# johnnyjana730/MVIN

Hardware: AMD Instinct MI355X
Metric: (user,item) pairs scored/sec @ dim=64 hop=2 fan-out=32; % HBM roofline (higher is better)
Workload: dtype f32

## Files before the change

mvin_amd/csrc/mvin_abi.hip:

```cpp
#include <cstdlib>
#include <cstdarg>
#include <cstdio>
#include <string>

#include "mvin_kernels.h"
#include "mvin_fused_agg.h"

namespace {

thread_local std::string g_last_error;

int fail(int code, const char* fmt, ...) {
    char buf[512];
    va_list ap;
    va_start(ap, fmt);
    vsnprintf(buf, sizeof(buf), fmt, ap);
    va_end(ap);
    g_last_error = buf;
    return code;
}

int hip_result(hipError_t e, const char* what) {
    if (e == hipSuccess) return 0;
    fail((int)e, "%s: %s", what, hipGetErrorString(e));
    return (int)e;
}

bool bad_dim(int D) { return D < 4 || D > MVIN_MAX_DIM || (D & 3) != 0; }

size_t geom_sum(int B, int K, int from, int to) {
    size_t s = 0, p = 1;
    for (int e = 0; e <= to; ++e) {
        if (e >= from) s += p;
        p *= (size_t)K;
    }
    return s * (size_t)B;
}

struct EntityTableList {
    const float* E;
    int n_entity;
    hipStream_t st;
    hipError_t err = hipSuccess;
    int n = 0;
    mvin::EntityTableJob jobs[mvin::kEtMaxJobs];
    void add(const float* W, int w_nk, float* out) {
        if (n == mvin::kEtMaxJobs) flush();
        jobs[n++] = mvin::EntityTableJob{W, out, w_nk};
    }
    void flush() {
        if (n > 0 && err == hipSuccess) err = mvin::launch_entity_tables(E, n_entity, jobs, n, st);
        n = 0;
    }
};

int build_entity_tables(const char* who, const float* E, int n_entity, const float* relation_kge, int nR, float* er, const float* user_mlp_W,
                        int n_o, float* tw, const float* fold_blk, float* fold_tabs, void* stream) {
    const size_t tab = (size_t)n_entity * 64, DD = (size_t)64 * 64;
    EntityTableList l{E, n_entity, (hipStream_t)stream};
    if (er)
        for (int r = 0; r < nR; ++r) l.add(relation_kge + r * DD, 1, er + r * tab);
    if (tw)
        for (int j = 0; j < n_o; ++j) l.add(user_mlp_W + j * DD, 0, tw + j * tab);
    if (fold_tabs)
        for (int i = 0; i < 4; ++i) l.add(fold_blk + i * DD, 0, fold_tabs + i * tab);
    l.flush();
    return hip_result(l.err, who);
}

}

extern "C" {

int mvin_abi_version(void) { return MVIN_ABI_VERSION; }

int mvin_debug_read_trace(long long* host_dst, size_t n) {
    if (!host_dst) return -1;
    static const bool ka = getenv("MVIN_KA_TRACE") != nullptr;
    static const bool pk = getenv("MVIN_PACK_TRACE") != nullptr;
    if (getenv("MVIN_SMALL_TRACE")) return (int)mvin::small_read_trace(host_dst, n);
    if (getenv("MVIN_KAF_TRACE")) return (int)mvin::kaf_read_trace(host_dst, n);
    if (pk) return (int)mvin::pack_read_prof(host_dst, n);
    if (ka && getenv("MVIN_KA_TRACE")[0] == '2') return (int)mvin::kas_read_trace(host_dst, n);
    return (int)(ka ? mvin::ka_read_trace(host_dst, n) : mvin::split_read_trace(host_dst, n));
}

const char* mvin_last_error(void) { return g_last_error.c_str(); }

size_t mvin_ent_elems(int B, int K, int levels) { return geom_sum(B, K, 0, levels); }

size_t mvin_rel_elems(int B, int K, int levels) { return levels > 0 ? geom_sum(B, K, 1, levels) : 0; }

int mvin_expand_ids(const int32_t* adj_entity, const int32_t* adj_relation, const int64_t* items_i64,
                    const int32_t* items_i32, int B, int K, int levels, int n_entity,
                    int32_t* ent_out, int32_t* rel_out, void* stream) {
    if (!ent_out || (!items_i64 && !items_i32) || (items_i64 && items_i32))
        return fail(-1, "mvin_expand_ids: need ent_out and exactly one of items_i64/items_i32");
    if (levels > 0 && (!adj_entity || !adj_relation || !rel_out))
        return fail(-1, "mvin_expand_ids: null adjacency/rel_out with levels=%d", levels);
    if (B <= 0 || K <= 0 || levels < 0 || n_entity <= 0)
        return fail(-2, "mvin_expand_ids: bad sizes B=%d K=%d levels=%d n_entity=%d", B, K, levels, n_entity);
    return hip_result(mvin::launch_expand(adj_entity, adj_relation, items_i64, items_i32, B, K, levels,
                                          n_entity, ent_out, rel_out, (hipStream_t)stream),
                      "mvin_expand_ids");
}

int mvin_rel_score(const float* relation_emb, const float* urh_weights, int nR, int D, float* t_out,
                   void* stream) {
    if (!relation_emb || !urh_weights || !t_out) return fail(-1, "mvin_rel_score: null pointer");
    if (nR <= 0 || D <= 0) return fail(-2, "mvin_rel_score: bad sizes nR=%d D=%d", nR, D);
    return hip_result(mvin::launch_rel_score(relation_emb, urh_weights, nR, D, t_out, (hipStream_t)stream),
                      "mvin_rel_score");
}

int mvin_linear_fwd(const mvin_linear_args* a, void* stream) {
    if (!a) return fail(-1, "mvin_linear_fwd: null args");
    if (a->nsrc < 1 || a->nsrc > MVIN_MAX_SRC) return fail(-2, "mvin_linear_fwd: nsrc=%d", a->nsrc);
    if (a->Dsrc < 4 || (a->Dsrc & 3) || a->Dout < 1 || a->Dout > MVIN_MAX_DIM)
        return fail(-2, "mvin_linear_fwd: Dsrc=%d (need %%4==0) Dout=%d (need 1..%d)", a->Dsrc, a->Dout,
                    MVIN_MAX_DIM);
    if ((size_t)a->nsrc * a->Dsrc > 4096) return fail(-2, "mvin_linear_fwd: nsrc*Dsrc > 4096");
    if (a->rows < 0) return fail(-2, "mvin_linear_fwd: rows < 0");
    if (!a->out) return fail(-1, "mvin_linear_fwd: null out");
    for (int s = 0; s < a->nsrc; ++s)
        if (!a->src[s]) return fail(-1, "mvin_linear_fwd: null src[%d]", s);
    if (!a->W && ((a->nsrc != 1 && !a->sum_sources) || a->Dsrc != a->Dout))
        return fail(-2, "mvin_linear_fwd: identity (W=NULL) needs nsrc==1 and Dsrc==Dout");
    if (a->ldo < a->Dout) return fail(-2, "mvin_linear_fwd: ldo < Dout");
    if (a->rowbias && a->rows_per_group < 1) return fail(-2, "mvin_linear_fwd: rows_per_group < 1");
    if (a->score_u && a->Dout > (a->sum_sources ? 1 : a->nsrc) * a->Dsrc + 4)
        return fail(-2, "mvin_linear_fwd: fused score needs Dout <= Din + 4");
    if (a->rows == 0) return 0;
    return hip_result(mvin::launch_linear(*a, (hipStream_t)stream), "mvin_linear_fwd");
}

static int agg_common(mvin::GatherAttnArgs& g, int B, int N, int K, int D, const char* who) {
    if (B <= 0 || N <= 0 || K <= 0) return fail(-2, "%s: bad sizes B=%d N=%d K=%d", who, B, N, K);
    if (bad_dim(D)) return fail(-2, "%s: D=%d (need %%4==0, 4..%d)", who, D, MVIN_MAX_DIM);
    if (K > 4096) return fail(-2, "%s: K=%d > 4096", who, K);
    if (!g.self_vec || !g.Wagg || !g.out) return fail(-1, "%s: null self_vec/Wagg/out", who);
    g.T = (int64_t)B * N;
    g.N = N;
    g.K = K;
    g.D = D;
    g.lpr_log2 = mvin::lpr_log2_for(D);
    return 0;
}

int mvin_gather_attn_fwd(const float* table, const int32_t* adj_entity, const int32_t* adj_relation,
                         const int32_t* node_ids, const float* rel_score, const float* self_vec,
                         const float* Wc, const float* c_child, const float* Wagg, const float* bagg, int B,
                         int N, int K, int D, int n_entity, float* out, float* probs, void* stream) {
    return mvin_gather_attn_fwd_ex(table, adj_entity, adj_relation, node_ids, rel_score, self_vec, Wc, c_child,
                                   Wagg, bagg, B, N, K, D, n_entity, out, probs, nullptr, nullptr, 0, stream);
}

int mvin_gather_attn_fwd_ex(const void* table, const int32_t* adj_entity, const int32_t* adj_relation,
                            const int32_t* node_ids, const float* rel_score, const float* self_vec,
                            const float* Wc, const float* c_child, const float* Wagg, const float* bagg, int B,
                            int N, int K, int D, int n_entity, float* out, float* probs, float* s_out,
                            float* z_out, int table_bf16, void* stream) {
    mvin::GatherAttnArgs g{};
    g.table_bf16 = table_bf16 ? 1 : 0;
    g.s_out = s_out;
    g.z_out = z_out;
    g.gather = 1;
    g.table = table;
    g.adj_e = adj_entity;
    g.adj_r = adj_relation;
    g.node_ids = node_ids;
    g.rel_score = rel_score;
    g.self_vec = self_vec;
    g.Wc = Wc;
    g.c_child = c_child;
    g.Wagg = Wagg;
    g.bagg = bagg;
    g.out = out;
    g.probs = probs;
    if (!table || !adj_entity || !node_ids || (rel_score && !adj_relation))
        return fail(-1, "mvin_gather_attn_fwd: null table/adjacency/node_ids");
    if (n_entity <= 0) return fail(-2, "mvin_gather_attn_fwd: n_entity=%d", n_entity);
    if (probs && !rel_score) return fail(-2, "mvin_gather_attn_fwd: probs requested without rel_score");
    if (int rc = agg_common(g, B, N, K, D, "mvin_gather_attn_fwd")) return rc;
    return hip_result(mvin::launch_gather_attn(g, (hipStream_t)stream), "mvin_gather_attn_fwd_ex");
}

int mvin_gather_attn_l2_supported(int D, int K) { return mvin::fused_l2_supported(D, K) ? 1 : 0; }

int mvin_probe_gather_l2(const void* table, const int32_t* child_ids, const int32_t* grandchild_ids, int64_t n_parents, int K,
                         int D, int n_entity, int table_bf16, float* sums, void* stream) {
    const char* who = "mvin_probe_gather_l2";
    if (!table || !child_ids || !grandchild_ids || !sums) return fail(-1, "%s: null pointer", who);
    if (n_parents <= 0 || K <= 0 || n_entity <= 0) return fail(-2, "%s: bad sizes", who);
    const int rb = D * (table_bf16 ? 2 : 4);
    if (!(rb == 64 || rb == 128 || rb == 256 || (rb == 512 && !table_bf16)))
        return fail(-3, "%s: row bytes %d (64, 128, 256 or 512)", who, rb);
    return hip_result(mvin::launch_gather_probe_l2(table, child_ids, grandchild_ids, n_parents, K, D, table_bf16, sums,
                                                   (hipStream_t)stream), who);
}

int mvin_gather_attn_l2_variant(int D, int K, int64_t n_parents, int n_entity, int want_probs) {
    return mvin_gather_attn_l2_variant_ex(D, K, n_parents, n_entity, want_probs, 0);
}

int mvin_gather_attn_l2_variant_ex(int D, int K, int64_t n_parents, int n_entity, int want_probs, int table_bf16) {
    if (!mvin::fused_l2_supported(D, K)) return 0;
    mvin::FusedL2Args f{};
    f.K = K;
    f.P = n_parents;
    f.adj_bytes = (uint64_t)n_entity * (uint64_t)K * 4;
    float probe = 0.f;
    if (want_probs) f.probs_parent = f.probs_child = &probe;
    f.table_bytes = (uint64_t)n_entity * (uint64_t)D * (table_bf16 ? 2 : 4);
    if (mvin::fused_d32_applies(f, D)) return 4;
    if (mvin::fused_l2_split_in_use() && mvin::fused_split_applies(f, D)) return 2;
    return mvin::fused_d16_applies(f, D) ? 3 : 1;
}

static int gather_attn_l2_impl(const void* table, const int32_t* adj_entity, const int32_t* adj_relation,
                               const int32_t* parent_ids, int pid_stride, const float* t0, const float* t1,
                               const float* W1, const float* W2, const float* b1, const float* b2, const float* q,
                               const float* A0, const float* a0, int B, int parents_per_pair, int K, int D,
                               int n_entity, int nR, float* nagg0, float* nagg1, float* probs_parent,
                               float* probs_child, int table_bf16, void* stream, bool encoded = false, bool prj = false,
                               const int32_t* order = nullptr, const float* agg = nullptr) {
    const char* who = prj ? "mvin_gather_attn_l2_prj_fwd" : encoded ? "mvin_gather_attn_l2_enc_fwd" : "mvin_gather_attn_l2_fwd";
    if (prj && (table_bf16 || !W1 || !W2 || !q))
        return fail(-1, "%s: projected tables are fp32 and go with the queries", who);
    if (encoded && !mvin::fused_packed_supported(D, K))
        return fail(-3, "%s: unsupported shape D=%d K=%d (D in {32,64,128}, K in {16,32,64,128})", who, D, K);
    if (!mvin::fused_l2_supported(D, K))
        return fail(-3, "%s: unsupported shape D=%d K=%d (D in {16,32,64,128}, K power of two in [4,256])",
                    who, D, K);
    if (!table || !adj_entity || !parent_ids || !A0 || !nagg0 || !nagg1) return fail(-1, "%s: null pointer", who);
    if ((t0 || t1) && !adj_relation) return fail(-1, "%s: attention needs adj_relation", who);
    if ((W1 == nullptr) != (W2 == nullptr)) return fail(-1, "%s: W1 and W2 must be given together", who);
    if (W1 && !q) return fail(-1, "%s: projection needs the query vectors q", who);
    if ((probs_parent || probs_child) && !t0) return fail(-2, "%s: probs requested without t0", who);
    if (B <= 0 || parents_per_pair <= 0 || n_entity <= 0 || nR <= 0 || nR > 4096)
        return fail(-2, "%s: bad sizes B=%d parents_per_pair=%d n_entity=%d nR=%d", who, B, parents_per_pair,
                    n_entity, nR);
    mvin::FusedL2Args f{};
    f.table = table;
    f.adj_e = adj_entity;
    f.adj_r = adj_relation;
    f.parent_ids = parent_ids;
    f.t0 = t0;
    f.t1 = t1;
    f.W1 = W1;
    f.W2 = W2;
    f.b1 = b1;
    f.b2 = b2;
    f.q = q;
    f.A0 = A0;
    f.a0 = a0;
    f.nagg0 = nagg0;
    f.nagg1 = nagg1;
    f.probs_parent = probs_parent;
    f.probs_child = probs_child;
    f.P = (int64_t)B * parents_per_pair;
    f.table_bytes = (uint64_t)n_entity * (uint64_t)D * (table_bf16 ? 2 : 4);
    f.adj_bytes = (uint64_t)n_entity * (uint64_t)K * 4;
    f.parents_per_pair = parents_per_pair;
    f.K = K;
    f.nR = nR;
    f.pid_stride = pid_stride;
    f.max_id = (unsigned)(n_entity - 1);
    f.prj = prj ? 1 : 0;
    int l = 0;
    if (agg) {
        f.agg = const_cast<float*>(agg);
        f.order = order;
        if (!(prj && encoded && mvin::fused_agg_applies(f, D) && (!order || parents_per_pair == 1)))
            return fail(-3, "mvin_gather_attn_l2_agg_fwd: D = 64, K in {16, 32, 64}, n_entity <= 2^24, tables < 1 GiB, adjacency and outputs < 2 GiB "
                            "(a parent order: one parent per pair)");
        return hip_result(mvin::launch_gather_attn_l2_agg(f, (hipStream_t)stream), "mvin_gather_attn_l2_agg_fwd");
    }
    if (order) {
        f.order = order;
        if (!(prj && encoded && parents_per_pair == 1 && mvin::fused_wpp_applies(f, D)))
            return fail(-3, "%s: a parent order is taken by the wave-per-parent kernel only (projected tables, encoded adjacency, D = 64, K <= 32, "
                            "one parent per pair)", who);
    }
    while ((4 << l) < K) ++l;
    f.lpn_log2 = l;
    {
        static const char* dbg = getenv("MVIN_SPLIT_DBG");
        f.dbg = dbg ? atoi(dbg) : 0;
    }
    if (prj && !encoded) {
        if (!mvin::fused_d32_applies(f, D)) return fail(-3, "%s: the projected-tables form over a plain adjacency exists for D = 32, K in {8, 16}", who);
        return hip_result(mvin::launch_gather_attn_l2_d32(f, 0, (hipStream_t)stream, false), who);
    }
    if (encoded) {
        if (!adj_relation) return fail(-1, "%s: null enc_relation", who);
        if (!mvin::fused_packed_applies(f, D))
            return fail(-3, "%s: tables too large (n_entity <= 2^24, table < 4 GiB, adjacency and outputs < 2 GiB)", who);
        static const bool d32enc_off = getenv("MVIN_L2_D32ENC") && atoi(getenv("MVIN_L2_D32ENC")) == 0;
        if (!d32enc_off && mvin::fused_d32_applies(f, D))
            return hip_result(mvin::launch_gather_attn_l2_d32(f, table_bf16, (hipStream_t)stream, true), who);
        if (prj && mvin::fused_wpp_applies(f, D)) return hip_result(mvin::launch_gather_attn_l2_wpp(f, (hipStream_t)stream), who);
        return hip_result(mvin::launch_gather_attn_l2_packed(f, D, table_bf16, (hipStream_t)stream), who);
    }
    return hip_result(mvin::launch_gather_attn_l2(f, D, table_bf16, (hipStream_t)stream), who);
}

int mvin_gather_attn_l2_enc_supported(int D, int K) { return mvin::fused_packed_supported(D, K) ? 1 : 0; }

int mvin_gather_attn_l2_enc_fwd(const void* table, const int32_t* enc_entity, const int32_t* enc_relation,
                                const void* parent_ids, int parent_ids_i64, const float* t0, const float* t1,
                                const float* W1, const float* W2, const float* b1, const float* b2, const float* q,
                                const float* A0, const float* a0, int B, int parents_per_pair, int K, int D, int n_entity,
                                int nR, float* nagg0, float* nagg1, int table_bf16, void* stream) {
    return gather_attn_l2_impl(table, enc_entity, enc_relation, reinterpret_cast<const int32_t*>(parent_ids),
                               parent_ids_i64 ? 2 : 1, t0, t1, W1, W2, b1, b2, q, A0, a0, B, parents_per_pair, K, D, n_entity,
                               nR, nagg0, nagg1, nullptr, nullptr, table_bf16, stream, true);
}

static int prj_linear(const float* src, int64_t rows, int D, const float* W1, const float* W2, const float* b1, const float* b2,
                      float* out, void* stream) {
    mvin_linear_args l{};
    l.src[0] = src;
    l.nsrc = 1;
    l.Dsrc = D;
    l.Dout = D;
    l.rows = rows;
    l.rows_per_group = 1;
    l.W = W1;
    l.w_zstride = W2 - W1;
    l.bias = b1;
    l.bias_zstride = b1 ? b2 - b1 : 0;
    l.out = out;
    l.ldo = D;
    l.nz = 2;
    l.out_zstride = rows * D;
    return mvin_linear_fwd(&l, stream);
}

int mvin_project_rows(const float* src, int64_t rows, int D, const float* W1, const float* W2, const float* b1, const float* b2,
                      float* out, void* stream) {
    const char* who = "mvin_project_rows";
    if (!src || !W1 || !W2 || !out) return fail(-1, "%s: null pointer", who);
    if ((b1 == nullptr) != (b2 == nullptr)) return fail(-1, "%s: b1 and b2 go together", who);
    if (rows <= 0 || D <= 0) return fail(-2, "%s: rows=%lld D=%d", who, (long long)rows, D);
    return prj_linear(src, rows, D, W1, W2, b1, b2, out, stream);
}

size_t mvin_project_tables_elems(int n_entity, int D) {
    if (n_entity <= 0 || D <= 0) return 0;
    return (size_t)3 * n_entity * D + (size_t)4 * D * D + (size_t)2 * D;
}

int mvin_project_tables(const float* entity_emb, const float* W1, const float* W2, const float* b1, const float* b2, const float* A0,
                        const float* a0, int attention, int K, int n_entity, int D, float* ws, void* stream) {
    const char* who = "mvin_project_tables";
    if (!entity_emb || !W1 || !W2 || !A0 || !ws) return fail(-1, "%s: null pointer", who);
    if ((b1 == nullptr) != (b2 == nullptr)) return fail(-1, "%s: b1 and b2 go together", who);
    if (n_entity <= 0 || K <= 0 || (D != 32 && D != 64 && D != 128)) return fail(-2, "%s: n_entity=%d K=%d D=%d", who, n_entity, K, D);
    float* blk = ws + (size_t)3 * n_entity * D;
    const float c = attention ? 1.f / (float)K : 1.f;
    if (int rc = hip_result(mvin::launch_prj_prepare(W1, W2, b1, b2, A0, a0, c, D, blk, (hipStream_t)stream), who)) return rc;
    mvin_linear_args l{};
    l.src[0] = entity_emb;
    l.nsrc = 1;
    l.Dsrc = D;
    l.Dout = D;
    l.rows = n_entity;
    l.rows_per_group = 1;
    l.W = blk;
    l.w_zstride = (int64_t)D * D;
    l.out = ws;
    l.ldo = D;
    l.nz = 3;
    l.out_zstride = (int64_t)n_entity * D;
    return mvin_linear_fwd(&l, stream);
}

static bool prj_applies(int D, int K, bool encoded, int n_entity, int nR, int64_t n_parents) {
    if (n_entity <= 0 || nR <= 0 || nR > 4096 || !mvin::fused_l2_supported(D, K)) return false;
    mvin::FusedL2Args f{};
    f.K = K;
    f.nR = nR;
    f.P = n_parents > 0 ? n_parents : 1;
    f.prj = 1;
// ... 1466 lines not shown
```

mvin_amd/csrc/mvin_fused_agg.h:

```cpp
#pragma once
#include <cstdlib>
#include <type_traits>

#include "mvin_kernels.h"

namespace mvin {

typedef float f32x4 __attribute__((ext_vector_type(4)));
typedef float f32x2 __attribute__((ext_vector_type(2)));
typedef unsigned int u32x4 __attribute__((ext_vector_type(4)));
typedef unsigned int u32x2 __attribute__((ext_vector_type(2)));

constexpr int kAggWaves = 4;
constexpr int kAggUvLd = 132;
constexpr int kAggPad = 4;
constexpr unsigned kAggOob = 0xFFFFFFF0u;
constexpr unsigned kAggPadRow = 0xFFFFFE00u;
constexpr int agg_list_words(int K) { return 4 * 2 * (K + kAggPad); }
size_t fused_agg_lds_bytes(int nR, int K);

__device__ __forceinline__ int agg_xor16_imax(int v) {
    const auto a = __builtin_amdgcn_permlane16_swap((unsigned)v, (unsigned)v, false, false);
    return max((int)a[0], (int)a[1]);
}
__device__ __forceinline__ int agg_xor32_imax(int v) {
    const auto a = __builtin_amdgcn_permlane32_swap((unsigned)v, (unsigned)v, false, false);
    return max((int)a[0], (int)a[1]);
}

__device__ __forceinline__ bool agg_logit_table(const float* t, int nR, float* sT, int tid, int lane) {
    float mx = -INFINITY, mn = INFINITY;
    if (t)
        for (int i = lane; i < nR; i += 64) {
            const float l = t[i];
            mx = fmaxf(mx, l), mn = fminf(mn, l);
        }
    else
        mx = mn = 0.f;
    mx = wave_max(mx), mn = -wave_max(-mn);
    const bool fast = __builtin_amdgcn_readfirstlane((mx - mn <= 60.f) ? 1 : 0) != 0;
    for (int i = tid; i < nR; i += kAggWaves * 64) {
        const float l = t ? t[i] : 0.f;
        sT[i] = fast ? lean_exp(fminf(l - mx, 0.f)) : l;
    }
    return fast;
}

template <int SPL, bool FAST, int LG = 4>
__device__ __forceinline__ void agg_row_weights(const unsigned (&cr)[SPL], bool att, const float* sT, float invK, float (&wk)[SPL]) {
    float lg[SPL];
    float mx = -INFINITY;
#pragma unroll
    for (int i = 0; i < SPL; ++i) {
        const float mu = (float)((cr[i] >> 16) & 0xFFu);
        const float l = att ? sT[cr[i] & 0xFFFFu] : (FAST ? 1.f : 0.f);
        if constexpr (FAST) {
            wk[i] = mu * l;
        } else {
            wk[i] = mu;
            mx = fmaxf(mx, mu > 0.f ? l : -INFINITY);
            lg[i] = l;
        }
    }
    if (att) {
        float z = 0.f;
        if constexpr (FAST) {
#pragma unroll
            for (int i = 0; i < SPL; ++i) z += wk[i];
        } else {
            mx = group_max(mx, LG);
#pragma unroll
            for (int i = 0; i < SPL; ++i) {
                wk[i] *= lean_exp(fminf(lg[i] - mx, 0.f));
                z += wk[i];
            }
        }
        z = group_sum(z, LG);
        const float rz = z > 0.f ? invK * __builtin_amdgcn_rcpf(z) : 0.f;
#pragma unroll
        for (int i = 0; i < SPL; ++i) wk[i] *= rz;
    } else {
#pragma unroll
        for (int i = 0; i < SPL; ++i) wk[i] *= invK;
    }
}

template <int SPL>
__device__ __forceinline__ void agg_load_slots(__amdgpu_buffer_rsrc_t adjE, __amdgpu_buffer_rsrc_t adjR, unsigned co, unsigned (&ce)[SPL],
                                               unsigned (&cr)[SPL]) {
    if constexpr (SPL == 1) {
        ce[0] = __builtin_amdgcn_raw_buffer_load_b32(adjE, co, 0, 0);
        cr[0] = __builtin_amdgcn_raw_buffer_load_b32(adjR, co, 0, 0);
    } else if constexpr (SPL == 2) {
        const u32x2 e2 = __builtin_amdgcn_raw_buffer_load_b64(adjE, co, 0, 0);
        const u32x2 r2 = __builtin_amdgcn_raw_buffer_load_b64(adjR, co, 0, 0);
        ce[0] = e2[0], ce[1] = e2[1], cr[0] = r2[0], cr[1] = r2[1];
    } else {
        static_assert(SPL == 4, "SPL");
        const u32x4 e4 = __builtin_amdgcn_raw_buffer_load_b128(adjE, co, 0, 0);
        const u32x4 r4 = __builtin_amdgcn_raw_buffer_load_b128(adjR, co, 0, 0);
#pragma unroll
        for (int i = 0; i < 4; ++i) ce[i] = e4[i], cr[i] = r4[i];
    }
}

__device__ __forceinline__ float4 agg_row4(__amdgpu_buffer_rsrc_t tab, unsigned off) {
    const u32x4 r = __builtin_amdgcn_raw_buffer_load_b128(tab, off, 0, 0);
    return make_float4(__uint_as_float(r[0]), __uint_as_float(r[1]), __uint_as_float(r[2]), __uint_as_float(r[3]));
}


struct FoldArgs {
    const float* agg;
    const float* M0;
    const int32_t* adj_e;
    const int32_t* adj_r;
    const int32_t* items;
    const float* t1;
    const float* q;
    const float* user_o;
    const float *Wq, *bq, *Wv, *bv, *Wqm, *A1, *a1, *Wm1, *Wm2, *bm;
    float* item_emb;
    float* scores;
    float* sig;
    int64_t B;
    uint64_t table_bytes, adj_bytes;
    int K, nR, pid_stride;
    unsigned max_id;
    int dbg;
    const float* tables;
    const float* t0;
    const int32_t* order;
};

hipError_t launch_entity_aggregates_d32(const EntityAggArgs& a, hipStream_t st);
hipError_t launch_score_l2_folded_d32(const FoldArgs& f, hipStream_t st);
hipError_t launch_score_l2_folded_gather(const FoldArgs& f, hipStream_t st);
size_t fused_wppfold_lds_bytes(int nR, int K);

}
```

mvin_amd/csrc/mvin_fused_agg.hip:

```cpp
#include "mvin_fused_agg.h"

namespace mvin {

template <int K>
__global__ __launch_bounds__(kAggWaves * 64) void entity_aggregates_kernel(EntityAggArgs a) {
    constexpr int D = 64, SPL = K / 16;
    static_assert(K == 16 || K == 32 || K == 64, "K");
    extern __shared__ __attribute__((aligned(16))) float smem[];
    const int nRp = (a.nR + 3) & ~3;
    float* sT = smem;
    const int tid = threadIdx.x, lane = tid & 63, wave = tid >> 6;
    const int g = lane >> 4, c = lane & 15;
    unsigned* sLo = reinterpret_cast<unsigned*>(sT + nRp + wave * agg_list_words(K)) + g * (K + kAggPad);
    float* sLw = reinterpret_cast<float*>(reinterpret_cast<unsigned*>(sT + nRp + wave * agg_list_words(K)) + 4 * (K + kAggPad)) + g * (K + kAggPad);
    const bool att = a.t0 != nullptr;
    const float invK = 1.f / (float)K;
    const bool fast = agg_logit_table(a.t0, a.nR, sT, tid, lane);
    __syncthreads();

    const int tbytes = (int)a.table_bytes;
    const __amdgpu_buffer_rsrc_t tabS = __builtin_amdgcn_make_buffer_rsrc(const_cast<float*>(a.tabS), 0, tbytes, 0x00020000);
    const __amdgpu_buffer_rsrc_t tabG = __builtin_amdgcn_make_buffer_rsrc(const_cast<float*>(a.tabG), 0, tbytes, 0x00020000);
    const __amdgpu_buffer_rsrc_t selfS = __builtin_amdgcn_make_buffer_rsrc(const_cast<float*>(a.selfS), 0, a.selfS ? tbytes : 0, 0x00020000);
    const __amdgpu_buffer_rsrc_t selfG = __builtin_amdgcn_make_buffer_rsrc(const_cast<float*>(a.selfG), 0, tbytes, 0x00020000);
    const __amdgpu_buffer_rsrc_t adjE = __builtin_amdgcn_make_buffer_rsrc(const_cast<int32_t*>(a.adj_e), 0, (int)a.adj_bytes, 0x00020000);
    const __amdgpu_buffer_rsrc_t adjR = __builtin_amdgcn_make_buffer_rsrc(const_cast<int32_t*>(a.adj_r), 0, (int)a.adj_bytes, 0x00020000);
    const __amdgpu_buffer_rsrc_t outS = __builtin_amdgcn_make_buffer_rsrc(a.outS, 0, tbytes, 0x00020000);
    const __amdgpu_buffer_rsrc_t outG = __builtin_amdgcn_make_buffer_rsrc(a.outG, 0, tbytes, 0x00020000);
    const unsigned c16 = (unsigned)c * 16u;
    const unsigned n_entity = (unsigned)a.n_entity;
    const unsigned nquad = (n_entity + 3u) >> 2;

    auto run = [&](auto fast_tag) {
        constexpr bool FAST = decltype(fast_tag)::value;
        for (unsigned quad = blockIdx.x * kAggWaves + wave; quad < nquad; quad += gridDim.x * kAggWaves) {
            const unsigned e = quad * 4u + (unsigned)g;
            const bool valid = e < n_entity;
            unsigned ce[SPL], cr[SPL];
            agg_load_slots<SPL>(adjE, adjR, valid ? (e * (unsigned)K + (unsigned)(SPL * c)) * 4u : kAggOob, ce, cr);
            const unsigned so = valid ? e * (unsigned)(D * 4) + c16 : kAggPadRow;
            const float4 sg = agg_row4(selfG, so);
            const float4 ss = agg_row4(selfS, so);
            float wk[SPL];
            agg_row_weights<SPL, FAST>(cr, att, sT, invK, wk);
            int cc = (int)(cr[0] >> 24);
            cc = valid ? (cc < 1 ? 1 : (cc > K ? K : cc)) : 0;
            __builtin_amdgcn_fence(__ATOMIC_RELEASE, "wavefront");
            __builtin_amdgcn_wave_barrier();
#pragma unroll
            for (int i = 0; i < SPL; ++i) {
                sLo[SPL * c + i] = ((cr[i] >> 16) & 0xFFu) ? (ce[i] & 0xFFFFFFu) * (unsigned)(D * 4) : kAggPadRow;
                sLw[SPL * c + i] = wk[i];
            }
            __builtin_amdgcn_fence(__ATOMIC_RELEASE, "wavefront");
            __builtin_amdgcn_wave_barrier();
            __builtin_amdgcn_fence(__ATOMIC_ACQUIRE, "wavefront");
            const int kmax = __builtin_amdgcn_readfirstlane(agg_xor32_imax(agg_xor16_imax(cc)));
            f32x2 s01 = {0.f, 0.f}, s23 = {0.f, 0.f}, g01 = {0.f, 0.f}, g23 = {0.f, 0.f};
            for (int k0 = 0; k0 < kmax; k0 += 4) {
                const uint4 o4 = *reinterpret_cast<const uint4*>(sLo + k0);
                const float4 w4 = *reinterpret_cast<const float4*>(sLw + k0);
                const unsigned off[4] = {o4.x, o4.y, o4.z, o4.w};
                const float ws_[4] = {w4.x, w4.y, w4.z, w4.w};
                float4 r1[4], r2[4];
#pragma unroll
                for (int t = 0; t < 4; ++t) {
                    r1[t] = agg_row4(tabS, off[t] + c16);
                    r2[t] = agg_row4(tabG, off[t] + c16);
                }
#pragma unroll
                for (int t = 0; t < 4; ++t) {
                    const f32x2 w2 = {ws_[t], ws_[t]};
                    s01 = __builtin_elementwise_fma(w2, f32x2{r1[t].x, r1[t].y}, s01);
                    s23 = __builtin_elementwise_fma(w2, f32x2{r1[t].z, r1[t].w}, s23);
                    g01 = __builtin_elementwise_fma(w2, f32x2{r2[t].x, r2[t].y}, g01);
                    g23 = __builtin_elementwise_fma(w2, f32x2{r2[t].z, r2[t].w}, g23);
                }
            }
            const unsigned oo = valid ? e * (unsigned)(D * 4) + c16 : kAggOob;
            const u32x4 vs = {__float_as_uint(s01[0] + ss.x), __float_as_uint(s01[1] + ss.y), __float_as_uint(s23[0] + ss.z),
                              __float_as_uint(s23[1] + ss.w)};
            const u32x4 vg = {__float_as_uint(g01[0] + sg.x), __float_as_uint(g01[1] + sg.y), __float_as_uint(g23[0] + sg.z),
                              __float_as_uint(g23[1] + sg.w)};
            __builtin_amdgcn_raw_buffer_store_b128(vs, outS, oo, 0, 0);
            __builtin_amdgcn_raw_buffer_store_b128(vg, outG, oo, 0, 0);
        }
    };
    if (fast) run(std::true_type{});
    else run(std::false_type{});
}

template <int K>
__global__ __launch_bounds__(kAggWaves * 64, K == 64 ? 3 : 4) void gather_attn_l2_agg_kernel(FusedL2Args a) {
    constexpr int D = 64, SPL = K / 16;
    static_assert(K == 16 || K == 32 || K == 64, "K");
    extern __shared__ __attribute__((aligned(16))) float smem[];
    const int nRp = (a.nR + 3) & ~3;
    float* sT = smem;
    const int tid = threadIdx.x, lane = tid & 63, wave = tid >> 6;
    const int g = lane >> 4, c = lane & 15;
    float* sUV = sT + nRp + wave * (16 * kAggUvLd + agg_list_words(K));
    unsigned* sLo = reinterpret_cast<unsigned*>(sUV + 16 * kAggUvLd) + g * (K + kAggPad);
    float* sLw = reinterpret_cast<float*>(reinterpret_cast<unsigned*>(sUV + 16 * kAggUvLd) + 4 * (K + kAggPad)) + g * (K + kAggPad);
    const bool att1 = a.t1 != nullptr;
    const float invK = 1.f / (float)K;
    const bool fold = a.fold != 0;
    const float c0 = fold ? 1.f : a.t0 != nullptr ? invK : 1.f;
    const bool fast = agg_logit_table(a.t1, a.nR, sT, tid, lane);
    __syncthreads();

    const unsigned tbytes = (unsigned)a.table_bytes;
    const __amdgpu_buffer_rsrc_t aggS = __builtin_amdgcn_make_buffer_rsrc(a.agg, 0, (int)tbytes, 0x00020000);
    const __amdgpu_buffer_rsrc_t aggG = __builtin_amdgcn_make_buffer_rsrc(reinterpret_cast<char*>(a.agg) + a.table_bytes, 0, (int)tbytes, 0x00020000);
    const __amdgpu_buffer_rsrc_t adjE = __builtin_amdgcn_make_buffer_rsrc(const_cast<int32_t*>(a.adj_e), 0, (int)a.adj_bytes, 0x00020000);
    const __amdgpu_buffer_rsrc_t adjR = __builtin_amdgcn_make_buffer_rsrc(const_cast<int32_t*>(a.adj_r), 0, (int)a.adj_bytes, 0x00020000);
    const __amdgpu_buffer_rsrc_t out0 = __builtin_amdgcn_make_buffer_rsrc(a.nagg0, 0, (int)(a.P * D * 4), 0x00020000);
    const __amdgpu_buffer_rsrc_t out1 = __builtin_amdgcn_make_buffer_rsrc(a.nagg1, 0, (int)(a.P * D * 4), 0x00020000);
    const unsigned c16 = (unsigned)c * 16u;
    if (c < kAggPad) {
        sLo[K + c] = kAggPadRow;
        sLw[K + c] = 0.f;
    }

    const int64_t nbatch = (a.P + 15) >> 4;
    const int64_t nwaves = (int64_t)gridDim.x * kAggWaves;
    auto run = [&](auto fast_tag) {
        constexpr bool FAST = decltype(fast_tag)::value;
        for (int64_t batch = (int64_t)blockIdx.x * kAggWaves + wave; batch < nbatch; batch += nwaves) {
            const int64_t p_base = batch << 4;
            int64_t pr = min(p_base + c, a.P - 1);
            if (a.order) pr = a.order[pr];
            const int x0c = fused_parent_id(a, pr);
            {
                const unsigned qoff = (unsigned)(pr / a.parents_per_pair) * (unsigned)(D * 4) + (unsigned)g * 16u;
                const char* qbase = reinterpret_cast<const char*>(a.q);
                float4 qb[4];
#pragma unroll
                for (int nt = 0; nt < 4; ++nt) qb[nt] = *reinterpret_cast<const float4*>(qbase + 64 * nt + (size_t)qoff);
                unsigned woff = ((unsigned)(4 * g) * (unsigned)D + (unsigned)c) * 4u;
                unsigned boff = (unsigned)g * 16u;
                asm volatile("" : "+v"(woff), "+v"(boff));
#pragma unroll
                for (int mat = 0; mat < 2; ++mat) {
                    const char* W = reinterpret_cast<const char*>(mat == 0 ? a.W1 : a.W2);
                    const char* bias = reinterpret_cast<const char*>(mat == 0 ? a.b1 : a.b2);
                    f32x4 acc[4];
#pragma unroll
                    for (int ntp = 0; ntp < 4; ++ntp) {
                        const float4 b = bias ? *reinterpret_cast<const float4*>(bias + 64 * ntp + (size_t)boff) : make_float4(0.f, 0.f, 0.f, 0.f);
                        acc[ntp] = f32x4{b.x, b.y, b.z, b.w};
                    }
#pragma unroll
                    for (int nt = 0; nt < 4; ++nt) {
                        const float bv[4] = {qb[nt].x, qb[nt].y, qb[nt].z, qb[nt].w};
#pragma unroll
                        for (int r = 0; r < 4; ++r) {
#pragma unroll
                            for (int ntp = 0; ntp < 4; ++ntp) {
                                const float w = *reinterpret_cast<const float*>(W + ((16 * nt + r) * D + 16 * ntp) * 4 + (size_t)woff);
                                acc[ntp] = __builtin_amdgcn_mfma_f32_16x16x4f32(w, bv[r], acc[ntp], 0, 0, 0);
                            }
                        }
                    }
#pragma unroll
                    for (int ntp = 0; ntp < 4; ++ntp)
                        *reinterpret_cast<float4*>(sUV + c * kAggUvLd + mat * D + 16 * ntp + 4 * g) = make_float4(acc[ntp][0], acc[ntp][1], acc[ntp][2], acc[ntp][3]);
                }
            }
            __builtin_amdgcn_fence(__ATOMIC_RELEASE, "wavefront");
            __builtin_amdgcn_wave_barrier();
            __builtin_amdgcn_fence(__ATOMIC_ACQUIRE, "wavefront");

            const int nquad = (int)((min((int64_t)16, a.P - p_base) + 3) >> 2);
            struct Quad {
                unsigned p;
                unsigned ce[SPL], cr[SPL];
                float4 s0;
            };
            auto quad_load = [&](int it) -> Quad {
                Quad qd;
                const int src = ((lane & 48) + 4 * it + g) << 2;
                qd.p = (unsigned)__builtin_amdgcn_ds_bpermute(src, (int)pr);
                const unsigned x0 = (unsigned)__builtin_amdgcn_ds_bpermute(src, x0c);
                agg_load_slots<SPL>(adjE, adjR, (x0 * (unsigned)K + (unsigned)(SPL * c)) * 4u, qd.ce, qd.cr);
                qd.s0 = agg_row4(aggS, x0 * (unsigned)(D * 4) + c16);
                return qd;
            };
            Quad nx = quad_load(0);
            for (int it = 0; it < nquad; ++it) {
                const int j = 4 * it + g;
                const bool pvalid = p_base + j < a.P;
                const Quad qd = nx;
                if (it + 1 < nquad) nx = quad_load(it + 1);
                const unsigned p = qd.p;
                const unsigned (&ce)[SPL] = qd.ce;
                const unsigned (&cr)[SPL] = qd.cr;
                const float4 s0 = qd.s0;
                const float4 u1 = *reinterpret_cast<const float4*>(sUV + j * kAggUvLd + 4 * c);
                const float4 vv = *reinterpret_cast<const float4*>(sUV + j * kAggUvLd + D + 4 * c);
                float wk[SPL];
                agg_row_weights<SPL, FAST>(cr, att1, sT, invK, wk);
                int cc = (int)(cr[0] >> 24);
                cc = pvalid ? (cc < 1 ? 1 : (cc > K ? K : cc)) : 0;
                __builtin_amdgcn_fence(__ATOMIC_RELEASE, "wavefront");
                __builtin_amdgcn_wave_barrier();
#pragma unroll
                for (int i = 0; i < SPL; ++i) {
                    sLo[SPL * c + i] = ((cr[i] >> 16) & 0xFFu) ? (ce[i] & 0xFFFFFFu) * (unsigned)(D * 4) : kAggPadRow;
                    sLw[SPL * c + i] = wk[i];
                }
                __builtin_amdgcn_fence(__ATOMIC_RELEASE, "wavefront");
                __builtin_amdgcn_wave_barrier();
                __builtin_amdgcn_fence(__ATOMIC_ACQUIRE, "wavefront");
                const int kmax = __builtin_amdgcn_readfirstlane(agg_xor32_imax(agg_xor16_imax(cc)));
                const f32x2 v01 = {vv.x, vv.y}, v23 = {vv.z, vv.w};
                f32x2 a01 = {0.f, 0.f}, a23 = {0.f, 0.f};
                float4 ra[4], rb[4];
                float4 wa, wb;
                auto issue = [&](int k, float4 (&r)[4], float4& w) {
                    const uint4 o4 = *reinterpret_cast<const uint4*>(sLo + k);
                    w = *reinterpret_cast<const float4*>(sLw + k);
                    r[0] = agg_row4(aggG, o4.x + c16), r[1] = agg_row4(aggG, o4.y + c16);
                    r[2] = agg_row4(aggG, o4.z + c16), r[3] = agg_row4(aggG, o4.w + c16);
                };
                auto sum4 = [&](const float4 (&r)[4], const float4& w) {
                    const float ws_[4] = {w.x, w.y, w.z, w.w};
#pragma unroll
                    for (int t = 0; t < 4; ++t) {
                        const f32x2 o01 = f32x2{r[t].x, r[t].y} + v01, o23 = f32x2{r[t].z, r[t].w} + v23;
                        const f32x2 w2 = {ws_[t], ws_[t]};
                        a01 = __builtin_elementwise_fma(w2, f32x2{fmaxf(o01[0], 0.f), fmaxf(o01[1], 0.f)}, a01);
                        a23 = __builtin_elementwise_fma(w2, f32x2{fmaxf(o23[0], 0.f), fmaxf(o23[1], 0.f)}, a23);
                    }
                };
                issue(0, ra, wa);
                for (int k0 = 0; k0 < kmax; k0 += 8) {
                    issue(k0 + 4, rb, wb);
                    __builtin_amdgcn_sched_barrier(0);
                    sum4(ra, wa);
                    __builtin_amdgcn_sched_barrier(0);
                    issue(k0 + 8, ra, wa);
                    __builtin_amdgcn_sched_barrier(0);
                    sum4(rb, wb);
                    __builtin_amdgcn_sched_barrier(0);
                }
                const unsigned oo = pvalid ? p * (unsigned)(D * 4) + c16 : kAggOob;
                float4 r0 = make_float4(fmaf(c0, u1.x, s0.x), fmaf(c0, u1.y, s0.y), fmaf(c0, u1.z, s0.z), fmaf(c0, u1.w, s0.w));
                float4 r1 = make_float4(a01[0], a01[1], a23[0], a23[1]);
                if (fold) {
                    r0 = make_float4(fmaxf(r0.x, 0.f), fmaxf(r0.y, 0.f), fmaxf(r0.z, 0.f), fmaxf(r0.w, 0.f));
                    r1 = make_float4(r1.x + r0.x, r1.y + r0.y, r1.z + r0.z, r1.w + r0.w);
                }
                const u32x4 o0 = {__float_as_uint(r0.x), __float_as_uint(r0.y), __float_as_uint(r0.z), __float_as_uint(r0.w)};
                const u32x4 o1 = {__float_as_uint(r1.x), __float_as_uint(r1.y), __float_as_uint(r1.z), __float_as_uint(r1.w)};
                __builtin_amdgcn_raw_buffer_store_b128(o0, out0, oo, 0, 0);
                __builtin_amdgcn_raw_buffer_store_b128(o1, out1, oo, 0, 0);
            }
            __builtin_amdgcn_fence(__ATOMIC_RELEASE, "wavefront");
            __builtin_amdgcn_wave_barrier();
            __builtin_amdgcn_fence(__ATOMIC_ACQUIRE, "wavefront");
        }
    };
    if (fast) run(std::true_type{});
    else run(std::false_type{});
}

template <int K>
__global__ __launch_bounds__(kAggWaves * 64, 3) void score_l2_folded_kernel(FoldArgs a) {
    constexpr int D = 64, SPL = K / 16;
    static_assert(K == 16 || K == 32 || K == 64, "K");
    extern __shared__ __attribute__((aligned(16))) float smem[];
    const int nRp = (a.nR + 3) & ~3;
    float* sT = smem;
    const int tid = threadIdx.x, lane = tid & 63, wave = tid >> 6;
    const int g = lane >> 4, c = lane & 15;
    float* sUV = sT + nRp + wave * (16 * kAggUvLd + agg_list_words(K));
    unsigned* sLo = reinterpret_cast<unsigned*>(sUV + 16 * kAggUvLd) + g * (K + kAggPad);
    float* sLw = reinterpret_cast<float*>(reinterpret_cast<unsigned*>(sUV + 16 * kAggUvLd) + 4 * (K + kAggPad)) + g * (K + kAggPad);
    const bool att1 = a.t1 != nullptr;
    const float invK = 1.f / (float)K;
    const bool fast = agg_logit_table(a.t1, a.nR, sT, tid, lane);
    __syncthreads();

    const int tbytes = (int)a.table_bytes;
    const __amdgpu_buffer_rsrc_t aggS = __builtin_amdgcn_make_buffer_rsrc(const_cast<float*>(a.agg), 0, tbytes, 0x00020000);
    const __amdgpu_buffer_rsrc_t aggG = __builtin_amdgcn_make_buffer_rsrc(reinterpret_cast<char*>(const_cast<float*>(a.agg)) + a.table_bytes, 0, tbytes, 0x00020000);
    const __amdgpu_buffer_rsrc_t adjE = __builtin_amdgcn_make_buffer_rsrc(const_cast<int32_t*>(a.adj_e), 0, (int)a.adj_bytes, 0x00020000);
    const __amdgpu_buffer_rsrc_t adjR = __builtin_amdgcn_make_buffer_rsrc(const_cast<int32_t*>(a.adj_r), 0, (int)a.adj_bytes, 0x00020000);
    const unsigned c16 = (unsigned)c * 16u;
    if (c < kAggPad) {
        sLo[K + c] = kAggPadRow;
        sLw[K + c] = 0.f;
    }

    const int64_t nbatch = (a.B + 15) >> 4;
    const int64_t nwaves = (int64_t)gridDim.x * kAggWaves;
    auto run = [&](auto fast_tag) {
        constexpr bool FAST = decltype(fast_tag)::value;
        for (int64_t batch = (int64_t)blockIdx.x * kAggWaves + wave; batch < nbatch; batch += nwaves) {
            const int64_t p_base = batch << 4;
            const int64_t pr = min(p_base + c, a.B - 1);
            const bool cvalid = p_base + c < a.B;
            unsigned x0u = (unsigned)a.items[pr * a.pid_stride];
            x0u = x0u < a.max_id ? x0u : a.max_id;
            const int x0c = (int)x0u;
            unsigned woff = ((unsigned)(4 * g) * (unsigned)D + (unsigned)c * 4u) * 4u;
            unsigned boff = (unsigned)g * 16u;
            unsigned roff = (unsigned)pr * (unsigned)(D * 4) + (unsigned)g * 16u;
            asm volatile("" : "+v"(woff), "+v"(boff));
            auto chain3 = [&](const float* W0p, const float* W1p, const float* W2p, const f32x4 (&b0)[4], const f32x4 (&b1)[4], const f32x4 (&b2)[4],
                              f32x4 (&acc0)[4], f32x4 (&acc1)[4], f32x4 (&acc2)[4], auto&& between) {
                asm volatile("" : "+s"(W0p), "+s"(W1p), "+s"(W2p));
                const __amdgpu_buffer_rsrc_t wr[3] = {__builtin_amdgcn_make_buffer_rsrc(const_cast<float*>(W0p), 0, D * D * 4, 0x00020000),
                                                      __builtin_amdgcn_make_buffer_rsrc(const_cast<float*>(W1p), 0, D * D * 4, 0x00020000),
                                                      __builtin_amdgcn_make_buffer_rsrc(const_cast<float*>(W2p), 0, D * D * 4, 0x00020000)};
                f32x4 ring[3][4];
                auto load = [&](auto s_) {
                    constexpr int s = decltype(s_)::value, j = s / 4, nt = s % 4;
#pragma unroll
                    for (int r = 0; r < 4; ++r) {
                        const u32x4 v = __builtin_amdgcn_raw_buffer_load_b128(wr[j], woff + (unsigned)(r * D * 4), nt * 16 * D * 4, 0);
                        ring[s % 3][r] = f32x4{__uint_as_float(v[0]), __uint_as_float(v[1]), __uint_as_float(v[2]), __uint_as_float(v[3])};
                    }
                };
                load(std::integral_constant<int, 0>{});
                load(std::integral_constant<int, 1>{});
                static_for<12>([&](auto s_) {
                    constexpr int s = decltype(s_)::value, j = s / 4, nt = s % 4;
                    if constexpr (s + 2 < 12) load(std::integral_constant<int, s + 2>{});
                    __builtin_amdgcn_sched_barrier(0);
                    const f32x4 (&b)[4] = j == 0 ? b0 : j == 1 ? b1 : b2;
                    f32x4 (&acc)[4] = j == 0 ? acc0 : j == 1 ? acc1 : acc2;
#pragma unroll
                    for (int r = 0; r < 4; ++r) {
#pragma unroll
                        for (int ntp = 0; ntp < 4; ++ntp) acc[ntp] = __builtin_amdgcn_mfma_f32_16x16x4f32(ring[s % 3][r][ntp], b[nt][r], acc[ntp], 0, 0, 0);
                    }
                    __builtin_amdgcn_sched_barrier(0);
                    if constexpr (nt == 3) between(std::integral_constant<int, j>{});
                });
            };
            auto bias4 = [&](const float* bp, f32x4 (&acc)[4]) {
                const char* bias = reinterpret_cast<const char*>(bp);
#pragma unroll
                for (int ntp = 0; ntp < 4; ++ntp)
                    acc[ntp] = bias ? *reinterpret_cast<const f32x4*>(bias + 64 * ntp + (size_t)boff) : f32x4{0.f, 0.f, 0.f, 0.f};
            };
            f32x4 qm[4], qb[4];
            {
                const char* qbase = reinterpret_cast<const char*>(a.q);
#pragma unroll
                for (int nt = 0; nt < 4; ++nt) qb[nt] = *reinterpret_cast<const f32x4*>(qbase + 64 * nt + (size_t)roff);
                f32x4 at[4], av[4];
                bias4(a.bq, at);
                bias4(a.bv, av);
                bias4(a.bm, qm);
                if (!(a.dbg & 4))
                    chain3(a.Wq, a.Wv, a.Wqm, qb, qb, qb, at, av, qm, [&](auto j_) {
                        constexpr int j = decltype(j_)::value;
                        if constexpr (j < 2) {
                            const f32x4 (&acc)[4] = j == 0 ? at : av;
#pragma unroll
                            for (int ntp = 0; ntp < 4; ++ntp) *reinterpret_cast<f32x4*>(sUV + c * kAggUvLd + j * D + 16 * ntp + 4 * g) = acc[ntp];
                        }
                    });
            }
            __builtin_amdgcn_fence(__ATOMIC_RELEASE, "wavefront");
            __builtin_amdgcn_wave_barrier();
            __builtin_amdgcn_fence(__ATOMIC_ACQUIRE, "wavefront");

            const int nquad = (a.dbg & 8) ? 0 : (int)((min((int64_t)16, a.B - p_base) + 3) >> 2);
            struct Quad {
                unsigned ce[SPL], cr[SPL];
                float4 s0;
            };
            auto quad_load = [&](int it) -> Quad {
                Quad qd;
                const unsigned x0 = (unsigned)__builtin_amdgcn_ds_bpermute(((lane & 48) + 4 * it + g) << 2, x0c);
                agg_load_slots<SPL>(adjE, adjR, (x0 * (unsigned)K + (unsigned)(SPL * c)) * 4u, qd.ce, qd.cr);
                qd.s0 = agg_row4(aggS, x0 * (unsigned)(D * 4) + c16);
                return qd;
            };
            Quad nx = quad_load(0);
            for (int it = 0; it < nquad; ++it) {
                const int j = 4 * it + g;
                const bool pvalid = p_base + j < a.B;
                const Quad qd = nx;
                if (it + 1 < nquad) nx = quad_load(it + 1);
                const unsigned (&ce)[SPL] = qd.ce;
                const unsigned (&cr)[SPL] = qd.cr;
                float* rowT = sUV + j * kAggUvLd + 4 * c;
                const float4 tt = *reinterpret_cast<const float4*>(rowT);
                const float4 vv = *reinterpret_cast<const float4*>(rowT + D);
                float wk[SPL];
                agg_row_weights<SPL, FAST>(cr, att1, sT, invK, wk);
                int cc = (int)(cr[0] >> 24);
                cc = pvalid ? (cc < 1 ? 1 : (cc > K ? K : cc)) : 0;
                __builtin_amdgcn_fence(__ATOMIC_RELEASE, "wavefront");
                __builtin_amdgcn_wave_barrier();
#pragma unroll
                for (int i = 0; i < SPL; ++i) {
                    sLo[SPL * c + i] = ((cr[i] >> 16) & 0xFFu) ? (ce[i] & 0xFFFFFFu) * (unsigned)(D * 4) : kAggPadRow;
                    sLw[SPL * c + i] = wk[i];
                }
                __builtin_amdgcn_fence(__ATOMIC_RELEASE, "wavefront");
                __builtin_amdgcn_wave_barrier();
                __builtin_amdgcn_fence(__ATOMIC_ACQUIRE, "wavefront");
                const int kmax = (a.dbg & 1) ? 0 : __builtin_amdgcn_readfirstlane(agg_xor32_imax(agg_xor16_imax(cc)));
                const f32x2 v01 = {vv.x, vv.y}, v23 = {vv.z, vv.w};
                f32x2 a01 = {0.f, 0.f}, a23 = {0.f, 0.f};
                float4 ra[4], rb[4];
                float4 wa, wb;
                auto issue = [&](int k, float4 (&r)[4], float4& w) {
                    const uint4 o4 = *reinterpret_cast<const uint4*>(sLo + k);
                    w = *reinterpret_cast<const float4*>(sLw + k);
                    r[0] = agg_row4(aggG, o4.x + c16), r[1] = agg_row4(aggG, o4.y + c16);
                    r[2] = agg_row4(aggG, o4.z + c16), r[3] = agg_row4(aggG, o4.w + c16);
                };
                auto sum4 = [&](const float4 (&r)[4], const float4& w) {
                    const float ws_[4] = {w.x, w.y, w.z, w.w};
#pragma unroll
                    for (int t = 0; t < 4; ++t) {
                        const f32x2 o01 = f32x2{r[t].x, r[t].y} + v01, o23 = f32x2{r[t].z, r[t].w} + v23;
                        const f32x2 w2 = {ws_[t], ws_[t]};
                        a01 = __builtin_elementwise_fma(w2, f32x2{fmaxf(o01[0], 0.f), fmaxf(o01[1], 0.f)}, a01);
                        a23 = __builtin_elementwise_fma(w2, f32x2{fmaxf(o23[0], 0.f), fmaxf(o23[1], 0.f)}, a23);
                    }
                };
                issue(0, ra, wa);
                for (int k0 = 0; k0 < kmax; k0 += 8) {
                    issue(k0 + 4, rb, wb);
                    __builtin_amdgcn_sched_barrier(0);
                    sum4(ra, wa);
                    __builtin_amdgcn_sched_barrier(0);
                    issue(k0 + 8, ra, wa);
                    __builtin_amdgcn_sched_barrier(0);
                    sum4(rb, wb);
                    __builtin_amdgcn_sched_barrier(0);
                }
                const float4 o0 = make_float4(fmaxf(qd.s0.x + tt.x, 0.f), fmaxf(qd.s0.y + tt.y, 0.f), fmaxf(qd.s0.z + tt.z, 0.f),
                                              fmaxf(qd.s0.w + tt.w, 0.f));
                *reinterpret_cast<float4*>(rowT) = o0;
                *reinterpret_cast<float4*>(rowT + D) = make_float4(a01[0] + o0.x, a01[1] + o0.y, a23[0] + o0.z, a23[1] + o0.w);
            }
            __builtin_amdgcn_fence(__ATOMIC_RELEASE, "wavefront");
            __builtin_amdgcn_wave_barrier();
            __builtin_amdgcn_fence(__ATOMIC_ACQUIRE, "wavefront");
            {
                f32x4 zb[4], ob[4], o2[4];
#pragma unroll
                for (int nt = 0; nt < 4; ++nt) zb[nt] = *reinterpret_cast<const f32x4*>(sUV + c * kAggUvLd + D + 16 * nt + 4 * g);
                bias4(a.a1, o2);
                if (!(a.dbg & 2))
                    chain3(a.A1, a.Wm1, a.Wm2, zb, ob, o2, o2, qm, qm, [&](auto j_) {
                        if constexpr (decltype(j_)::value == 0) {
#pragma unroll
                            for (int nt = 0; nt < 4; ++nt) {
                                o2[nt] = f32x4{fmaxf(o2[nt][0], 0.f), fmaxf(o2[nt][1], 0.f), fmaxf(o2[nt][2], 0.f), fmaxf(o2[nt][3], 0.f)};
                                ob[nt] = *reinterpret_cast<const f32x4*>(sUV + c * kAggUvLd + 16 * nt + 4 * g);
                            }
                        }
                    });
                const bool uo_is_q = a.user_o == a.q;
                float part = 0.f;
#pragma unroll
                for (int ntp = 0; ntp < 4; ++ntp) {
                    const f32x4 m0 = *reinterpret_cast<const f32x4*>(reinterpret_cast<const char*>(a.M0) + (size_t)x0u * (D * 4) + 64 * ntp + (size_t)boff);
                    const f32x4 uo = uo_is_q ? qb[ntp] : *reinterpret_cast<const f32x4*>(reinterpret_cast<const char*>(a.user_o) + 64 * ntp + (size_t)roff);
                    const f32x4 it4 = qm[ntp] + m0;
                    if (a.item_emb && cvalid) *reinterpret_cast<f32x4*>(reinterpret_cast<char*>(a.item_emb) + 64 * ntp + (size_t)roff) = it4;
                    part += it4[0] * uo[0] + it4[1] * uo[1] + it4[2] * uo[2] + it4[3] * uo[3];
                }
                part = xor32_sum(xor16_sum(part));
                if (g == 0 && cvalid) {
                    a.scores[pr] = part;
                    if (a.sig) a.sig[pr] = 1.f / (1.f + expf(-part));
                }
            }
            __builtin_amdgcn_fence(__ATOMIC_RELEASE, "wavefront");
            __builtin_amdgcn_wave_barrier();
            __builtin_amdgcn_fence(__ATOMIC_ACQUIRE, "wavefront");
        }
    };
    if (fast) run(std::true_type{});
    else run(std::false_type{});
}

template <int K>
static hipError_t launch_fold_k(const FoldArgs& a, hipStream_t st) {
    const size_t lds = fused_agg_lds_bytes(a.nR, K);
    static thread_local int per_cu = 0;
    if (per_cu == 0) {
        int v = 0;
        if (hipOccupancyMaxActiveBlocksPerMultiprocessor(&v, reinterpret_cast<const void*>(score_l2_folded_kernel<K>), kAggWaves * 64, lds) != hipSuccess || v < 1)
            v = 4;
        per_cu = v > 8 ? 8 : v;
        if (const char* e = getenv("MVIN_FOLD_WGS")) per_cu = atoi(e) > 0 ? atoi(e) : per_cu;
    }
    const int64_t nbatch = (a.B + 15) >> 4;
    const int64_t want = (nbatch + kAggWaves - 1) / kAggWaves;
    const int64_t cap = 256 * (int64_t)per_cu;
    score_l2_folded_kernel<K><<<(int)(want < cap ? want : cap), kAggWaves * 64, lds, st>>>(a);
    return hipGetLastError();
}

hipError_t launch_score_l2_folded(const float* agg, const float* M0, const int32_t* adj_e, const int32_t* adj_r, const int32_t* items, int pid_stride,
                                  const float* t1, const float* q, const float* user_o, const float* Wq, const float* bq, const float* Wv,
                                  const float* bv, const float* Wqm, const float* A1, const float* a1, const float* Wm1, const float* Wm2,
                                  const float* bm, float* item_emb, float* scores, float* sig, int64_t B, int K, int D, int nR, int n_entity,
                                  hipStream_t st) {
    FoldArgs f{};
    f.agg = agg, f.M0 = M0, f.adj_e = adj_e, f.adj_r = adj_r, f.items = items, f.pid_stride = pid_stride, f.t1 = t1, f.q = q, f.user_o = user_o;
    f.Wq = Wq, f.bq = bq, f.Wv = Wv, f.bv = bv, f.Wqm = Wqm, f.A1 = A1, f.a1 = a1, f.Wm1 = Wm1, f.Wm2 = Wm2, f.bm = bm;
    f.item_emb = item_emb, f.scores = scores, f.sig = sig, f.B = B, f.K = K, f.nR = nR, f.max_id = (unsigned)(n_entity - 1);
    f.table_bytes = (uint64_t)n_entity * (uint64_t)D * 4, f.adj_bytes = (uint64_t)n_entity * (uint64_t)K * 4;
    static const char* dbg = getenv("MVIN_FOLD_DBG");
    f.dbg = dbg ? atoi(dbg) : 0;
    if (D == 32) return launch_score_l2_folded_d32(f, st);
    switch (K) {
        case 16: return launch_fold_k<16>(f, st);
        case 32: return launch_fold_k<32>(f, st);
        case 64: return launch_fold_k<64>(f, st);
        default: return hipErrorInvalidValue;
    }
}

bool fused_agg_supported(int D, int K) { return D == 64 && (K == 16 || K == 32 || K == 64); }
bool fused_fold_supported(int D, int K) { return fused_agg_supported(D, K) || (D == 32 && (K == 16 || K == 32)); }
size_t fused_fold_d32_lds_bytes(int nR, int K);
size_t fused_fold_lds_bytes(int D, int nR, int K) { return D == 32 ? fused_fold_d32_lds_bytes(nR, K) : fused_agg_lds_bytes(nR, K); }

size_t fused_agg_lds_bytes(int nR, int K) {
    return ((size_t)((nR + 3) & ~3) + (size_t)kAggWaves * (16 * kAggUvLd + agg_list_words(K))) * sizeof(float);
}

bool fused_agg_applies(const FusedL2Args& a, int D) {
    return a.prj && fused_agg_supported(D, a.K) && !a.probs_parent && !a.probs_child && a.adj_r && a.adj_bytes > 0 &&
           a.adj_bytes < (1ull << 31) && a.table_bytes > 0 && a.table_bytes < (1ull << 30) && (uint64_t)a.P * D * 4 < (1ull << 31) &&
           a.max_id < (1u << 24) && a.nR > 0 && fused_agg_lds_bytes(a.nR, a.K) <= 48 * 1024;
}

template <int K>
static hipError_t launch_entity_aggregates_k(const EntityAggArgs& a, hipStream_t st) {
    const size_t lds = ((size_t)((a.nR + 3) & ~3) + (size_t)kAggWaves * agg_list_words(K)) * sizeof(float);
    const int64_t nquad = ((int64_t)a.n_entity + 3) >> 2;
    const int64_t want = (nquad + kAggWaves - 1) / kAggWaves;
    const int64_t cap = 256 * 8;
    entity_aggregates_kernel<K><<<(int)(want < cap ? want : cap), kAggWaves * 64, lds, st>>>(a);
    return hipGetLastError();
}

hipError_t launch_entity_aggregates(const EntityAggArgs& a, hipStream_t st) {
    if (a.D == 32) return launch_entity_aggregates_d32(a, st);
    switch (a.K) {
        case 16: return launch_entity_aggregates_k<16>(a, st);
        case 32: return launch_entity_aggregates_k<32>(a, st);
        case 64: return launch_entity_aggregates_k<64>(a, st);
        default: return hipErrorInvalidValue;
    }
}

__global__ void fold_prepare_kernel(const float* __restrict__ W0, const float* __restrict__ b0, const float* __restrict__ W1,
                                    const float* __restrict__ b1, const float* __restrict__ W2, const float* __restrict__ b2,
                                    const float* __restrict__ A0, const float* __restrict__ a0, const float* __restrict__ Wmix,
                                    const float* __restrict__ bmix, const float* __restrict__ A1, float c, int D, float* __restrict__ blk) {
    const int i = blockIdx.x, j = threadIdx.x;
    float* Wstack = blk;
    float* Wv = blk + (size_t)4 * D * D;
    float* Wq = Wv + (size_t)D * D;
    float* bv = Wq + (size_t)D * D;
    float* bq = bv + D;
    float* bm = bq + D;
    if (j >= D) return;
    float s0 = 0.f, s1 = 0.f, s2 = 0.f, sm = 0.f;
    for (int k0 = 0; k0 < D; k0 += 8) {
        float av[8], mv[8], x0[8], x1[8], x2[8];
#pragma unroll
        for (int k = 0; k < 8; ++k) {
            av[k] = A0[(size_t)(k0 + k) * D + j];
            mv[k] = Wmix[(size_t)(k0 + k) * D + j];
            x0[k] = i < D ? W0[(size_t)i * D + k0 + k] : (b0 ? b0[k0 + k] : 0.f);
            x1[k] = i < D ? W1[(size_t)i * D + k0 + k] : (b1 ? b1[k0 + k] : 0.f);
            x2[k] = i < D ? W2[(size_t)i * D + k0 + k] : (b2 ? b2[k0 + k] : 0.f);
        }
#pragma unroll
        for (int k = 0; k < 8; ++k) {
            s0 = fmaf(x0[k], av[k], s0);
            s1 = fmaf(x1[k], av[k], s1);
            s2 = fmaf(x2[k], av[k], s2);
            sm = fmaf(x0[k], mv[k], sm);
        }
    }
    if (i < D) {
        Wstack[(size_t)i * D + j] = s1;
        Wstack[(size_t)D * D + (size_t)i * D + j] = s2;
        Wstack[(size_t)2 * D * D + (size_t)i * D + j] = s0;
        Wstack[(size_t)3 * D * D + (size_t)i * D + j] = sm;
        Wv[(size_t)i * D + j] = fmaf(c, s2, s1);
        Wq[(size_t)i * D + j] = fmaf(c, s1, s0);
        if (D == 64 || D == 32) {
            float* Wperm = bm + D;
            const size_t o = (size_t)i * D + (size_t)(j & 15) * (D / 16) + (size_t)(j >> 4);
            const size_t DD = (size_t)D * D;
            Wperm[o] = fmaf(c, s1, s0);
            Wperm[DD + o] = fmaf(c, s2, s1);
            Wperm[2 * DD + o] = sm;
            Wperm[3 * DD + o] = A1[(size_t)i * D + j];
            Wperm[4 * DD + o] = Wmix[DD + (size_t)i * D + j];
            Wperm[5 * DD + o] = Wmix[2 * DD + (size_t)i * D + j];
        }
    } else {
        const float av0 = a0 ? a0[j] : 0.f;
        bv[j] = fmaf(c, s2, s1) + av0;
        bq[j] = fmaf(c, s1, s0) + av0;
        bm[j] = (bmix ? bmix[j] : 0.f) + sm;
    }
}

hipError_t launch_fold_prepare(const float* W0, const float* b0, const float* W1, const float* b1, const float* W2, const float* b2, const float* A0,
                               const float* a0, const float* Wmix, const float* bmix, const float* A1, float c, int D, float* blk, hipStream_t st) {
    fold_prepare_kernel<<<D + 1, D < 64 ? 64 : D, 0, st>>>(W0, b0, W1, b1, W2, b2, A0, a0, Wmix, bmix, A1, c, D, blk);
    return hipGetLastError();
}

template <int K>
static hipError_t launch_agg_k(const FusedL2Args& a, hipStream_t st) {
    const size_t lds = fused_agg_lds_bytes(a.nR, K);
    static thread_local int per_cu = 0;
    if (per_cu == 0) {
        int v = 0;
        if (hipOccupancyMaxActiveBlocksPerMultiprocessor(&v, reinterpret_cast<const void*>(gather_attn_l2_agg_kernel<K>), kAggWaves * 64, lds) != hipSuccess || v < 1)
            v = 4;
        per_cu = v > 8 ? 8 : v;
    }
    const int64_t nbatch = (a.P + 15) >> 4;
    const int64_t want = (nbatch + kAggWaves - 1) / kAggWaves;
    const int64_t cap = 256 * (int64_t)per_cu;
    gather_attn_l2_agg_kernel<K><<<(int)(want < cap ? want : cap), kAggWaves * 64, lds, st>>>(a);
    return hipGetLastError();
}

hipError_t launch_gather_attn_l2_agg(const FusedL2Args& a, hipStream_t st) {
    switch (a.K) {
        case 16: return launch_agg_k<16>(a, st);
        case 32: return launch_agg_k<32>(a, st);
        case 64: return launch_agg_k<64>(a, st);
        default: return hipErrorInvalidValue;
    }
}

}
```

mvin_amd/csrc/mvin_fused_agg32.hip:

```cpp
#include "mvin_fused_agg.h"

namespace mvin {

constexpr int kA32Ld = 68;
constexpr int a32_list_words(int K) { return 8 * 2 * (K + kAggPad); }

__device__ __forceinline__ int a32_groups_imax(int v) {
    const int m = __builtin_amdgcn_update_dpp(0, v, 0x140, 0xF, 0xF, true);
    return agg_xor32_imax(agg_xor16_imax(max(v, m)));
}

template <int K>
__global__ __launch_bounds__(kAggWaves * 64) void entity_aggregates_d32_kernel(EntityAggArgs a) {
    constexpr int D = 32, SPL = K / 8;
    static_assert(K == 16 || K == 32, "K");
    extern __shared__ __attribute__((aligned(16))) float smem[];
    const int nRp = (a.nR + 3) & ~3;
    float* sT = smem;
    const int tid = threadIdx.x, lane = tid & 63, wave = tid >> 6;
    const int g = lane >> 3, c = lane & 7;
    unsigned* sLo = reinterpret_cast<unsigned*>(sT + nRp + wave * a32_list_words(K)) + g * (K + kAggPad);
    float* sLw = reinterpret_cast<float*>(reinterpret_cast<unsigned*>(sT + nRp + wave * a32_list_words(K)) + 8 * (K + kAggPad)) + g * (K + kAggPad);
    const bool att = a.t0 != nullptr;
    const float invK = 1.f / (float)K;
    const bool fast = agg_logit_table(a.t0, a.nR, sT, tid, lane);
    __syncthreads();

    const int tbytes = (int)a.table_bytes;
    const __amdgpu_buffer_rsrc_t tabS = __builtin_amdgcn_make_buffer_rsrc(const_cast<float*>(a.tabS), 0, tbytes, 0x00020000);
    const __amdgpu_buffer_rsrc_t tabG = __builtin_amdgcn_make_buffer_rsrc(const_cast<float*>(a.tabG), 0, tbytes, 0x00020000);
    const __amdgpu_buffer_rsrc_t selfS = __builtin_amdgcn_make_buffer_rsrc(const_cast<float*>(a.selfS), 0, a.selfS ? tbytes : 0, 0x00020000);
    const __amdgpu_buffer_rsrc_t selfG = __builtin_amdgcn_make_buffer_rsrc(const_cast<float*>(a.selfG), 0, tbytes, 0x00020000);
    const __amdgpu_buffer_rsrc_t adjE = __builtin_amdgcn_make_buffer_rsrc(const_cast<int32_t*>(a.adj_e), 0, (int)a.adj_bytes, 0x00020000);
    const __amdgpu_buffer_rsrc_t adjR = __builtin_amdgcn_make_buffer_rsrc(const_cast<int32_t*>(a.adj_r), 0, (int)a.adj_bytes, 0x00020000);
    const __amdgpu_buffer_rsrc_t outS = __builtin_amdgcn_make_buffer_rsrc(a.outS, 0, tbytes, 0x00020000);
    const __amdgpu_buffer_rsrc_t outG = __builtin_amdgcn_make_buffer_rsrc(a.outG, 0, tbytes, 0x00020000);
    const unsigned c16 = (unsigned)c * 16u;
    const unsigned n_entity = (unsigned)a.n_entity;
    const unsigned noct = (n_entity + 7u) >> 3;

    auto run = [&](auto fast_tag) {
        constexpr bool FAST = decltype(fast_tag)::value;
        for (unsigned oct = blockIdx.x * kAggWaves + wave; oct < noct; oct += gridDim.x * kAggWaves) {
            const unsigned e = oct * 8u + (unsigned)g;
            const bool valid = e < n_entity;
            unsigned ce[SPL], cr[SPL];
            agg_load_slots<SPL>(adjE, adjR, valid ? (e * (unsigned)K + (unsigned)(SPL * c)) * 4u : kAggOob, ce, cr);
            const unsigned so = valid ? e * (unsigned)(D * 4) + c16 : kAggPadRow;
            const float4 sg = agg_row4(selfG, so);
            const float4 ss = agg_row4(selfS, so);
            float wk[SPL];
            agg_row_weights<SPL, FAST, 3>(cr, att, sT, invK, wk);
            int cc = (int)(cr[0] >> 24);
            cc = valid ? (cc < 1 ? 1 : (cc > K ? K : cc)) : 0;
            __builtin_amdgcn_fence(__ATOMIC_RELEASE, "wavefront");
            __builtin_amdgcn_wave_barrier();
#pragma unroll
            for (int i = 0; i < SPL; ++i) {
                sLo[SPL * c + i] = ((cr[i] >> 16) & 0xFFu) ? (ce[i] & 0xFFFFFFu) * (unsigned)(D * 4) : kAggPadRow;
                sLw[SPL * c + i] = wk[i];
            }
            __builtin_amdgcn_fence(__ATOMIC_RELEASE, "wavefront");
            __builtin_amdgcn_wave_barrier();
            __builtin_amdgcn_fence(__ATOMIC_ACQUIRE, "wavefront");
            const int kmax = __builtin_amdgcn_readfirstlane(a32_groups_imax(cc));
            f32x2 s01 = {0.f, 0.f}, s23 = {0.f, 0.f}, g01 = {0.f, 0.f}, g23 = {0.f, 0.f};
            for (int k0 = 0; k0 < kmax; k0 += 4) {
                const uint4 o4 = *reinterpret_cast<const uint4*>(sLo + k0);
                const float4 w4 = *reinterpret_cast<const float4*>(sLw + k0);
                const unsigned off[4] = {o4.x, o4.y, o4.z, o4.w};
                const float ws_[4] = {w4.x, w4.y, w4.z, w4.w};
                float4 r1[4], r2[4];
#pragma unroll
                for (int t = 0; t < 4; ++t) {
                    r1[t] = agg_row4(tabS, off[t] + c16);
                    r2[t] = agg_row4(tabG, off[t] + c16);
                }
#pragma unroll
                for (int t = 0; t < 4; ++t) {
                    const f32x2 w2 = {ws_[t], ws_[t]};
                    s01 = __builtin_elementwise_fma(w2, f32x2{r1[t].x, r1[t].y}, s01);
                    s23 = __builtin_elementwise_fma(w2, f32x2{r1[t].z, r1[t].w}, s23);
                    g01 = __builtin_elementwise_fma(w2, f32x2{r2[t].x, r2[t].y}, g01);
                    g23 = __builtin_elementwise_fma(w2, f32x2{r2[t].z, r2[t].w}, g23);
                }
            }
            const unsigned oo = valid ? e * (unsigned)(D * 4) + c16 : kAggOob;
            const u32x4 vs = {__float_as_uint(s01[0] + ss.x), __float_as_uint(s01[1] + ss.y), __float_as_uint(s23[0] + ss.z),
                              __float_as_uint(s23[1] + ss.w)};
            const u32x4 vg = {__float_as_uint(g01[0] + sg.x), __float_as_uint(g01[1] + sg.y), __float_as_uint(g23[0] + sg.z),
                              __float_as_uint(g23[1] + sg.w)};
            __builtin_amdgcn_raw_buffer_store_b128(vs, outS, oo, 0, 0);
            __builtin_amdgcn_raw_buffer_store_b128(vg, outG, oo, 0, 0);
        }
    };
    if (fast) run(std::true_type{});
    else run(std::false_type{});
}

template <int K>
__global__ __launch_bounds__(kAggWaves * 64, 3) void score_l2_folded_d32_kernel(FoldArgs a) {
    constexpr int D = 32, SPL = K / 8, NT = 2;
    static_assert(K == 16 || K == 32, "K");
    extern __shared__ __attribute__((aligned(16))) float smem[];
    const int nRp = (a.nR + 3) & ~3;
    float* sT = smem;
    const int tid = threadIdx.x, lane = tid & 63, wave = tid >> 6;
    const int g = lane >> 4, c = lane & 15;
    const int g8 = lane >> 3, c8 = lane & 7;
    float* sUV = sT + nRp + wave * (16 * kA32Ld + a32_list_words(K));
    unsigned* sLo = reinterpret_cast<unsigned*>(sUV + 16 * kA32Ld) + g8 * (K + kAggPad);
    float* sLw = reinterpret_cast<float*>(reinterpret_cast<unsigned*>(sUV + 16 * kA32Ld) + 8 * (K + kAggPad)) + g8 * (K + kAggPad);
    const bool att1 = a.t1 != nullptr;
    const float invK = 1.f / (float)K;
    const bool fast = agg_logit_table(a.t1, a.nR, sT, tid, lane);
    __syncthreads();

    const int tbytes = (int)a.table_bytes;
    const __amdgpu_buffer_rsrc_t aggS = __builtin_amdgcn_make_buffer_rsrc(const_cast<float*>(a.agg), 0, tbytes, 0x00020000);
    const __amdgpu_buffer_rsrc_t aggG = __builtin_amdgcn_make_buffer_rsrc(reinterpret_cast<char*>(const_cast<float*>(a.agg)) + a.table_bytes, 0, tbytes, 0x00020000);
    const __amdgpu_buffer_rsrc_t adjE = __builtin_amdgcn_make_buffer_rsrc(const_cast<int32_t*>(a.adj_e), 0, (int)a.adj_bytes, 0x00020000);
    const __amdgpu_buffer_rsrc_t adjR = __builtin_amdgcn_make_buffer_rsrc(const_cast<int32_t*>(a.adj_r), 0, (int)a.adj_bytes, 0x00020000);
    const unsigned c16 = (unsigned)c8 * 16u;
    if (c8 < kAggPad) {
        sLo[K + c8] = kAggPadRow;
        sLw[K + c8] = 0.f;
    }

    const int64_t nbatch = (a.B + 15) >> 4;
    const int64_t nwaves = (int64_t)gridDim.x * kAggWaves;
    auto run = [&](auto fast_tag) {
        constexpr bool FAST = decltype(fast_tag)::value;
        for (int64_t batch = (int64_t)blockIdx.x * kAggWaves + wave; batch < nbatch; batch += nwaves) {
            const int64_t p_base = batch << 4;
            const int64_t pr = min(p_base + c, a.B - 1);
            const bool cvalid = p_base + c < a.B;
            unsigned x0u = (unsigned)a.items[pr * a.pid_stride];
            x0u = x0u < a.max_id ? x0u : a.max_id;
            const int x0c = (int)x0u;
            unsigned woff = ((unsigned)(4 * g) * 16u + (unsigned)c) * (unsigned)(NT * 4);
            unsigned boff = (unsigned)g * 16u;
            unsigned roff = (unsigned)pr * (unsigned)(D * 4) + (unsigned)g * 16u;
            asm volatile("" : "+v"(woff), "+v"(boff));
            auto chain3 = [&](const float* W0p, const float* W1p, const float* W2p, const f32x4 (&b0)[NT], const f32x4 (&b1)[NT], const f32x4 (&b2)[NT],
                              f32x4 (&acc0)[NT], f32x4 (&acc1)[NT], f32x4 (&acc2)[NT], auto&& between) {
                asm volatile("" : "+s"(W0p), "+s"(W1p), "+s"(W2p));
                const __amdgpu_buffer_rsrc_t wr[3] = {__builtin_amdgcn_make_buffer_rsrc(const_cast<float*>(W0p), 0, D * D * 4, 0x00020000),
                                                      __builtin_amdgcn_make_buffer_rsrc(const_cast<float*>(W1p), 0, D * D * 4, 0x00020000),
                                                      __builtin_amdgcn_make_buffer_rsrc(const_cast<float*>(W2p), 0, D * D * 4, 0x00020000)};
                f32x2 ring[3][4];
                auto load = [&](auto s_) {
                    constexpr int s = decltype(s_)::value, j = s / NT, nt = s % NT;
#pragma unroll
                    for (int r = 0; r < 4; ++r) {
                        const u32x2 v = __builtin_amdgcn_raw_buffer_load_b64(wr[j], woff + (unsigned)(r * D * 4), nt * 16 * D * 4, 0);
                        ring[s % 3][r] = f32x2{__uint_as_float(v[0]), __uint_as_float(v[1])};
                    }
                };
                load(std::integral_constant<int, 0>{});
                load(std::integral_constant<int, 1>{});
                static_for<3 * NT>([&](auto s_) {
                    constexpr int s = decltype(s_)::value, j = s / NT, nt = s % NT;
                    if constexpr (s + 2 < 3 * NT) load(std::integral_constant<int, s + 2>{});
                    __builtin_amdgcn_sched_barrier(0);
                    const f32x4 (&b)[NT] = j == 0 ? b0 : j == 1 ? b1 : b2;
                    f32x4 (&acc)[NT] = j == 0 ? acc0 : j == 1 ? acc1 : acc2;
#pragma unroll
                    for (int r = 0; r < 4; ++r) {
#pragma unroll
                        for (int ntp = 0; ntp < NT; ++ntp) acc[ntp] = __builtin_amdgcn_mfma_f32_16x16x4f32(ring[s % 3][r][ntp], b[nt][r], acc[ntp], 0, 0, 0);
                    }
                    __builtin_amdgcn_sched_barrier(0);
                    if constexpr (nt == NT - 1) between(std::integral_constant<int, j>{});
                });
            };
            auto bias4 = [&](const float* bp, f32x4 (&acc)[NT]) {
                const char* bias = reinterpret_cast<const char*>(bp);
#pragma unroll
                for (int ntp = 0; ntp < NT; ++ntp)
                    acc[ntp] = bias ? *reinterpret_cast<const f32x4*>(bias + 64 * ntp + (size_t)boff) : f32x4{0.f, 0.f, 0.f, 0.f};
            };
            f32x4 qm[NT], qb[NT];
            {
                const char* qbase = reinterpret_cast<const char*>(a.q);
#pragma unroll
                for (int nt = 0; nt < NT; ++nt) qb[nt] = *reinterpret_cast<const f32x4*>(qbase + 64 * nt + (size_t)roff);
                f32x4 at[NT], av[NT];
                bias4(a.bq, at);
                bias4(a.bv, av);
                bias4(a.bm, qm);
                chain3(a.Wq, a.Wv, a.Wqm, qb, qb, qb, at, av, qm, [&](auto j_) {
                    constexpr int j = decltype(j_)::value;
                    if constexpr (j < 2) {
                        const f32x4 (&acc)[NT] = j == 0 ? at : av;
#pragma unroll
                        for (int ntp = 0; ntp < NT; ++ntp) *reinterpret_cast<f32x4*>(sUV + c * kA32Ld + j * D + 16 * ntp + 4 * g) = acc[ntp];
                    }
                });
            }
            __builtin_amdgcn_fence(__ATOMIC_RELEASE, "wavefront");
            __builtin_amdgcn_wave_barrier();
            __builtin_amdgcn_fence(__ATOMIC_ACQUIRE, "wavefront");

            const int noct = (int)((min((int64_t)16, a.B - p_base) + 7) >> 3);
            struct Oct {
                unsigned ce[SPL], cr[SPL];
                float4 s0;
            };
            auto oct_load = [&](int it) -> Oct {
                Oct qd;
                const unsigned x0 = (unsigned)__builtin_amdgcn_ds_bpermute(((lane & 48) + 8 * it + g8) << 2, x0c);
                agg_load_slots<SPL>(adjE, adjR, (x0 * (unsigned)K + (unsigned)(SPL * c8)) * 4u, qd.ce, qd.cr);
                qd.s0 = agg_row4(aggS, x0 * (unsigned)(D * 4) + c16);
                return qd;
            };
            Oct nx = oct_load(0);
            for (int it = 0; it < noct; ++it) {
                const int j = 8 * it + g8;
                const bool pvalid = p_base + j < a.B;
                const Oct qd = nx;
                if (it + 1 < noct) nx = oct_load(it + 1);
                const unsigned (&ce)[SPL] = qd.ce;
                const unsigned (&cr)[SPL] = qd.cr;
                float* rowT = sUV + j * kA32Ld + 4 * c8;
                const float4 tt = *reinterpret_cast<const float4*>(rowT);
                const float4 vv = *reinterpret_cast<const float4*>(rowT + D);
                float wk[SPL];
                agg_row_weights<SPL, FAST, 3>(cr, att1, sT, invK, wk);
                int cc = (int)(cr[0] >> 24);
                cc = pvalid ? (cc < 1 ? 1 : (cc > K ? K : cc)) : 0;
                __builtin_amdgcn_fence(__ATOMIC_RELEASE, "wavefront");
                __builtin_amdgcn_wave_barrier();
#pragma unroll
                for (int i = 0; i < SPL; ++i) {
                    sLo[SPL * c8 + i] = ((cr[i] >> 16) & 0xFFu) ? (ce[i] & 0xFFFFFFu) * (unsigned)(D * 4) : kAggPadRow;
                    sLw[SPL * c8 + i] = wk[i];
                }
                __builtin_amdgcn_fence(__ATOMIC_RELEASE, "wavefront");
                __builtin_amdgcn_wave_barrier();
                __builtin_amdgcn_fence(__ATOMIC_ACQUIRE, "wavefront");
                const int kmax = __builtin_amdgcn_readfirstlane(a32_groups_imax(cc));
                const f32x2 v01 = {vv.x, vv.y}, v23 = {vv.z, vv.w};
                f32x2 a01 = {0.f, 0.f}, a23 = {0.f, 0.f};
                float4 ra[4], rb[4];
                float4 wa, wb;
                auto issue = [&](int k, float4 (&r)[4], float4& w) {
                    const uint4 o4 = *reinterpret_cast<const uint4*>(sLo + k);
                    w = *reinterpret_cast<const float4*>(sLw + k);
                    r[0] = agg_row4(aggG, o4.x + c16), r[1] = agg_row4(aggG, o4.y + c16);
                    r[2] = agg_row4(aggG, o4.z + c16), r[3] = agg_row4(aggG, o4.w + c16);
                };
                auto sum4 = [&](const float4 (&r)[4], const float4& w) {
                    const float ws_[4] = {w.x, w.y, w.z, w.w};
#pragma unroll
                    for (int t = 0; t < 4; ++t) {
                        const f32x2 o01 = f32x2{r[t].x, r[t].y} + v01, o23 = f32x2{r[t].z, r[t].w} + v23;
                        const f32x2 w2 = {ws_[t], ws_[t]};
                        a01 = __builtin_elementwise_fma(w2, f32x2{fmaxf(o01[0], 0.f), fmaxf(o01[1], 0.f)}, a01);
                        a23 = __builtin_elementwise_fma(w2, f32x2{fmaxf(o23[0], 0.f), fmaxf(o23[1], 0.f)}, a23);
                    }
                };
                issue(0, ra, wa);
                for (int k0 = 0; k0 < kmax; k0 += 8) {
                    issue(k0 + 4, rb, wb);
                    __builtin_amdgcn_sched_barrier(0);
                    sum4(ra, wa);
                    __builtin_amdgcn_sched_barrier(0);
                    issue(k0 + 8, ra, wa);
                    __builtin_amdgcn_sched_barrier(0);
                    sum4(rb, wb);
                    __builtin_amdgcn_sched_barrier(0);
                }
                const float4 o0 = make_float4(fmaxf(qd.s0.x + tt.x, 0.f), fmaxf(qd.s0.y + tt.y, 0.f), fmaxf(qd.s0.z + tt.z, 0.f),
                                              fmaxf(qd.s0.w + tt.w, 0.f));
                *reinterpret_cast<float4*>(rowT) = o0;
                *reinterpret_cast<float4*>(rowT + D) = make_float4(a01[0] + o0.x, a01[1] + o0.y, a23[0] + o0.z, a23[1] + o0.w);
            }
            __builtin_amdgcn_fence(__ATOMIC_RELEASE, "wavefront");
            __builtin_amdgcn_wave_barrier();
            __builtin_amdgcn_fence(__ATOMIC_ACQUIRE, "wavefront");
            {
                f32x4 zb[NT], ob[NT], o2[NT];
#pragma unroll
                for (int nt = 0; nt < NT; ++nt) zb[nt] = *reinterpret_cast<const f32x4*>(sUV + c * kA32Ld + D + 16 * nt + 4 * g);
                bias4(a.a1, o2);
                chain3(a.A1, a.Wm1, a.Wm2, zb, ob, o2, o2, qm, qm, [&](auto j_) {
                    if constexpr (decltype(j_)::value == 0) {
#pragma unroll
                        for (int nt = 0; nt < NT; ++nt) {
                            o2[nt] = f32x4{fmaxf(o2[nt][0], 0.f), fmaxf(o2[nt][1], 0.f), fmaxf(o2[nt][2], 0.f), fmaxf(o2[nt][3], 0.f)};
                            ob[nt] = *reinterpret_cast<const f32x4*>(sUV + c * kA32Ld + 16 * nt + 4 * g);
                        }
                    }
                });
                const bool uo_is_q = a.user_o == a.q;
                float part = 0.f;
#pragma unroll
                for (int ntp = 0; ntp < NT; ++ntp) {
                    const f32x4 m0 = *reinterpret_cast<const f32x4*>(reinterpret_cast<const char*>(a.M0) + (size_t)x0u * (D * 4) + 64 * ntp + (size_t)boff);
                    const f32x4 uo = uo_is_q ? qb[ntp] : *reinterpret_cast<const f32x4*>(reinterpret_cast<const char*>(a.user_o) + 64 * ntp + (size_t)roff);
                    const f32x4 it4 = qm[ntp] + m0;
                    if (a.item_emb && cvalid) *reinterpret_cast<f32x4*>(reinterpret_cast<char*>(a.item_emb) + 64 * ntp + (size_t)roff) = it4;
                    part += it4[0] * uo[0] + it4[1] * uo[1] + it4[2] * uo[2] + it4[3] * uo[3];
                }
                part = xor32_sum(xor16_sum(part));
                if (g == 0 && cvalid) {
                    a.scores[pr] = part;
                    if (a.sig) a.sig[pr] = 1.f / (1.f + expf(-part));
                }
            }
            __builtin_amdgcn_fence(__ATOMIC_RELEASE, "wavefront");
            __builtin_amdgcn_wave_barrier();
            __builtin_amdgcn_fence(__ATOMIC_ACQUIRE, "wavefront");
        }
    };
    if (fast) run(std::true_type{});
    else run(std::false_type{});
}

size_t fused_fold_d32_lds_bytes(int nR, int K) {
    return ((size_t)((nR + 3) & ~3) + (size_t)kAggWaves * (16 * kA32Ld + a32_list_words(K))) * sizeof(float);
}

template <int K>
static hipError_t launch_ea32_k(const EntityAggArgs& a, hipStream_t st) {
    const size_t lds = ((size_t)((a.nR + 3) & ~3) + (size_t)kAggWaves * a32_list_words(K)) * sizeof(float);
    const int64_t noct = ((int64_t)a.n_entity + 7) >> 3;
    const int64_t want = (noct + kAggWaves - 1) / kAggWaves;
    const int64_t cap = 256 * 8;
    entity_aggregates_d32_kernel<K><<<(int)(want < cap ? want : cap), kAggWaves * 64, lds, st>>>(a);
    return hipGetLastError();
}

hipError_t launch_entity_aggregates_d32(const EntityAggArgs& a, hipStream_t st) {
    switch (a.K) {
        case 16: return launch_ea32_k<16>(a, st);
        case 32: return launch_ea32_k<32>(a, st);
        default: return hipErrorInvalidValue;
    }
}

template <int K>
static hipError_t launch_fold32_k(const FoldArgs& a, hipStream_t st) {
    const size_t lds = fused_fold_d32_lds_bytes(a.nR, K);
    static thread_local int per_cu = 0;
    if (per_cu == 0) {
        int v = 0;
        if (hipOccupancyMaxActiveBlocksPerMultiprocessor(&v, reinterpret_cast<const void*>(score_l2_folded_d32_kernel<K>), kAggWaves * 64, lds) != hipSuccess || v < 1)
            v = 3;
        per_cu = v > 8 ? 8 : v;
    }
    const int64_t nbatch = (a.B + 15) >> 4;
    const int64_t want = (nbatch + kAggWaves - 1) / kAggWaves;
    const int64_t cap = 256 * (int64_t)per_cu;
    score_l2_folded_d32_kernel<K><<<(int)(want < cap ? want : cap), kAggWaves * 64, lds, st>>>(a);
    return hipGetLastError();
}

hipError_t launch_score_l2_folded_d32(const FoldArgs& f, hipStream_t st) {
    switch (f.K) {
        case 16: return launch_fold32_k<16>(f, st);
        case 32: return launch_fold32_k<32>(f, st);
        default: return hipErrorInvalidValue;
    }
}

}
```

mvin_amd/csrc/mvin_kernels.h:

```cpp
#pragma once
#include <hip/hip_runtime.h>
#include <stdint.h>

#include "../../include/mvin_hip.h"
#include "mvin_common.h"

namespace mvin {

struct GatherAttnArgs {
    int gather;
    int table_bf16;
    const void* table;
    const int32_t* adj_e;
    const int32_t* adj_r;
    const int32_t* node_ids;
    const float* neigh;
    const int32_t* rel_ids;
    const float* rel_score;
    const float* self_vec;
    const float* Wc;
    const float* c_child;
    const float* Wagg;
    const float* bagg;
    float* out;
// ... 27 lines not shown
    const int32_t* hist_items;
    int32_t* out;
    int64_t n_user;
    uint64_t seed;
    int P, Nm, n_neighbor;
};

struct KeyAddrArgs {
    const void* E;
    const float* V;
    const float* w;
    const int32_t* mem_h[8];
    const int32_t* mem_r[8];
    const int32_t* mem_t[8];
    float* out;
    int64_t ldo;
    int64_t B;
    int P, Nm, D, nR, lpr_log2;
    uint64_t table_bytes;
    const int32_t* uts;
    const int64_t* users64;
    const int32_t* users32;
    int n_user;
    int n_entity;
};

struct KeyAddrLists {
    const int32_t *h, *r, *t;
};
__device__ __forceinline__ KeyAddrLists key_addr_lists(const KeyAddrArgs& a, int64_t b, int hop) {
    if (a.uts) {
        int64_t u = a.users64 ? a.users64[b] : (int64_t)a.users32[b];
        u = u < 0 ? 0 : (u >= a.n_user ? a.n_user - 1 : u);
        const int32_t* base = a.uts + ((u * (a.P > 0 ? a.P : 1) + hop) * 3) * (int64_t)a.Nm;
        return {base, base + a.Nm, base + 2 * a.Nm};
    }
    const int64_t o = b * a.Nm;
    return {a.mem_h[hop] + o, hop < a.P ? a.mem_r[hop] + o : nullptr, hop < a.P ? a.mem_t[hop] + o : nullptr};
}

struct KeyAddrGroupedArgs {
    const void* E;
    const float* R;
    const float* w;
    const int32_t* uts;
    const int32_t* seg_user;
    const int32_t* seg_ptr;
    const int32_t* nseg_dev;
    const int32_t* pair_index;
    const int64_t* items64;
    const int32_t* items32;
    float* out;
    int64_t ldo;
    int nseg, P, Nm, D, nR, NRL;
    int n_entity;
    int dbg;
    const int32_t* records;
    const float* ER;
    const float* hs;
};

struct KaFlashArgs {
    const float* E;
    const float* ER;
    const float* hs;
    const int32_t* records;
    const int32_t* seg_user;
    const int32_t* seg_ptr;
    const int32_t* nseg_dev;
    const int32_t* pair_index;
    const int64_t* items64;
    const int32_t* items32;
    const float* TW;
    const float* bmlp;
    float* user_o;
    int32_t* slot_seg;
    int32_t* counter;
    int nslots;
    int P, Nm, nR, n_entity;
    int64_t B;
};

struct KaRecLayout {
    int NmP, rows, maxtiles, o_cnt, o_off, o_trel, o_bidx, o_head, o_tail, o_hr, len;
};

struct TailArgs {
    const void* E;
    const int64_t* items64;
    const int32_t* items32;
    const float* q;
    const float* user_o;
    const float* nagg0;
    const float* nagg1;
    const float* W0;
    const float* b0;
    const float* A0;
    const float* a0;
    const float* A1;
    const float* a1;
    const float* Wmix;
    const float* bmix;
    float* item_emb;
    float* scores;
    float* sig;
    int64_t B;
    int table_bf16;
    int n_entity;
    int dbg;
};

struct EntityAggArgs {
    const float* tabS;
    const float* tabG;
    const float* selfS;
    const float* selfG;
    const int32_t* adj_e;
    const int32_t* adj_r;
    const float* t0;
    float* outS;
    float* outG;
    int n_entity, K, nR;
    uint64_t table_bytes, adj_bytes;
    int D;
};

struct TailFoldArgs {
    const float* M0;
    const int64_t* items64;
    const int32_t* items32;
    const float* q;
    const float* user_o;
    const float* out0;
    const float* z2;
    const float* Wqm;
    const float* A1;
    const float* a1;
    const float* Wmix;
    const float* bm;
    float* item_emb;
    float* scores;
    float* sig;
    int64_t B;
    int n_entity;
};

struct GatherMixArgs {
    const void* table;
    const int32_t* adj_e;
    const int32_t* adj_r;
    const int32_t* node_ids;
    const float* rel_score;
    const float* rowbias;
    float* out;
    int64_t nodes;
    int npg, K, D, lpr_log2, relu, table_bf16;
};

struct FusedL2Args {
    const void* table;
    const int32_t* adj_e;
    const int32_t* adj_r;
    const int32_t* parent_ids;
    const float* t0;
    const float* t1;
    const float* W1;
    const float* W2;
    const float* q;
    const float* b1;
    const float* b2;
    const float* A0;
    const float* a0;
    float* nagg0;
    float* nagg1;
    float* probs_parent;
    float* probs_child;
    int64_t P;
    uint64_t table_bytes;
    uint64_t adj_bytes;
    int parents_per_pair, K, nR, lpn_log2;
    int pid_stride;
    unsigned max_id;
    int dbg;
    const int32_t* order;
    float* agg;
    int fold;
    int prj;
};

__device__ __forceinline__ int fused_parent_id(const FusedL2Args& a, int64_t i) {
    const unsigned v = (unsigned)a.parent_ids[i * a.pid_stride];
    return (int)(v < a.max_id ? v : a.max_id);
}

struct EltArgs {
    int mode;
    int64_t n;
    float* x;
    float* y;
    float* z;
    float* w;
    float* accum;
    float alpha, beta, beta1, beta2, eps;
    int D, N;
};

struct WgradArgs {
    mvin_linear_args lin;
    const float* dY;
    int64_t ldy, dy_zstride;
    const float* mask;
    int64_t ldm, mask_zstride;
    float* dW;
    int64_t dw_zstride;
    float* db;
    int64_t db_zstride;
    int IB;
};

struct AggBwdArgs {
    int gather;
    const float* table;
    const int32_t* adj_e;
    const int32_t* adj_r;
    const int32_t* node_ids;
    const float* child;
    const int32_t* rel_ids;
    const float* probs;
    const float* rel_score;
    int skip_zero;
    const float* dvec;
    float* dtable;
    float* dchild;
    float* dT;
    int64_t T;
    int K, D, nR, lpr_log2;
};

struct KeyAddrBwdArgs {
    KeyAddrArgs f;
    const float* dout;
    float* dE;
    float* dV;
    float* dw;
    float l2;
    const float* Rk;
    const void* items;
    int items64;
    int dw_rep;
    int dv_lds;
    float* reg_accum;
};

hipError_t launch_eltwise(const EltArgs& a, hipStream_t st);
hipError_t launch_l2_adam_multi(const mvin_param_seg* segs, int nseg, int64_t total, float* g, float* mo, float* vo,
                                float* accum, int apply_adam, float lr_t, const float* lr_dev, float b1, float b2,
                                float eps, hipStream_t st);
hipError_t launch_scatter_add_rows(float* dtable, const int32_t* ids, int ids64, const float* x, int64_t rows, int D,
                                   float alpha, hipStream_t st);
hipError_t launch_linear_wgrad(WgradArgs a, hipStream_t st);
hipError_t launch_linear_wgrad_multi(const WgradArgs* probs, int n, hipStream_t st);
hipError_t launch_agg_bwd(const AggBwdArgs& a, hipStream_t st);
hipError_t launch_rel_score_bwd(const float* rel, const float* urh_w, const float* dT, int nR, int D, float* drel,
                                float* durh, hipStream_t st);
hipError_t launch_key_addr_bwd(const KeyAddrBwdArgs& a, hipStream_t st);

inline int lpr_log2_for(int D) {
    int l = 0;
    while ((4 << l) < D) ++l;
    return l;
}

hipError_t launch_expand(const int32_t* adj_e, const int32_t* adj_r, const int64_t* items64,
                         const int32_t* items32, int B, int K, int levels, int n_entity,
                         int32_t* ent_out, int32_t* rel_out, hipStream_t st);
hipError_t launch_rel_score(const float* rel, const float* urh_w, int nR, int D, float* t,
                            hipStream_t st);
hipError_t launch_linear(const mvin_linear_args& a, hipStream_t st);
bool linear_mfma_supported(const mvin_linear_args& a);
hipError_t launch_linear_mfma(const mvin_linear_args& a, hipStream_t st);
hipError_t launch_gather_attn(const GatherAttnArgs& a, hipStream_t st);
hipError_t launch_ripple(const RippleArgs& a, hipStream_t st);
hipError_t launch_sample_adjacency(const int64_t* indptr, const int32_t* dst, const int32_t* rel, int n_entity,
                                   int K, uint64_t seed, int32_t* adj_e, int32_t* adj_r, hipStream_t st);
hipError_t launch_ripple_build(const RippleBuildArgs& a, hipStream_t st);
int key_addr_nj(int Nm, int D);
bool key_addr_grouped_supported(int D, int P, int Nm, int nR);
hipError_t launch_key_addr_grouped(const KeyAddrGroupedArgs& a, int table_bf16, hipStream_t st);
bool key_addr_wave16_supported(int D, int P, int Nm, int nR);
bool key_addr_wave16_applies(const KeyAddrGroupedArgs& a);
hipError_t launch_key_addr_wave16(const KeyAddrGroupedArgs& a, int table_bf16, hipStream_t st);
bool key_addr_dense_supported(int D, int P, int Nm, int nR);
hipError_t launch_key_addr_dense(const KeyAddrGroupedArgs& a, int table_bf16, hipStream_t st);
KaRecLayout ka_rec_layout(int P, int Nm, int nR);
hipError_t launch_user_records(const int32_t* uts, int n_user, int P, int Nm, int nR, int n_entity, int32_t* out, hipStream_t st);
bool key_addr_static_supported(int D, int P, int Nm, int nR);
bool key_addr_static_applies(const KeyAddrGroupedArgs& a, int table_bf16);
hipError_t launch_key_addr_static(const KeyAddrGroupedArgs& a, hipStream_t st);
bool key_addr_flash_supported(int D, int P, int Nm, int nR, int n_entity);
size_t key_addr_flash_ws_elems(int64_t B, int nseg_bound);
hipError_t launch_key_addr_flash(const KaFlashArgs& a, int nseg_bound, bool has_set, int32_t* sched_ws, hipStream_t st);
hipError_t kas_read_trace(long long* host_dst, size_t n);
hipError_t kaf_read_trace(long long* host_dst, size_t n);
hipError_t launch_key_addr(const KeyAddrArgs& a, int table_bf16, hipStream_t st);
bool key_addr_stream_supported(const KeyAddrArgs& a, int table_bf16);
hipError_t launch_key_addr_stream(const KeyAddrArgs& a, int table_bf16, hipStream_t st);
hipError_t launch_move_rows(void* table, const int32_t* ids, int64_t n, int row_bytes, void* rows, bool scatter,
                            hipStream_t st);
hipError_t launch_shard_space_ids(const void* ids, bool is64, int64_t n, int world, int n_local, void* out, hipStream_t st);
hipError_t launch_row_softmax(const float* x, int64_t rows, int n, float* out, hipStream_t st);
hipError_t launch_mix_urv(const float* neigh, const float* rel, const float* user, const float* logits, int64_t nodes, int N, int K,
                          int D, float* out, float* probs, hipStream_t st);
hipError_t launch_gather_mix(const GatherMixArgs& a, hipStream_t st);
struct ScoreSmallArgs {
    const void* E;
    const int32_t* adj_e;
    const int32_t* adj_r;
    const float* R;
    const float* w_h;
    const float* Wu;
    const float* bu;
    const float* t0;
    const float* t1;
    const float *W0, *b0, *W1, *b1, *W2, *b2;
    const float *A0, *a0, *A1, *a1, *Wmix, *bmix;
    const int64_t* items;
    const int32_t* mem_h[4];
    const int32_t* mem_r[4];
    const int32_t* mem_t[4];
    const int32_t* uts;
    const int64_t* users;
    float* user_o;
    float* item_emb;
    float* scores;
    float* sig;
    int64_t B;
    int G;
    int K, P, Nm, nR, n_entity, n_user, enc, table_bf16;
    int depth1;
    int dbg;
    uint64_t table_bytes;
    uint64_t adj_bytes;
};
bool score_small_supported(int D, int K, int P, int Nm, int nR);
int score_small_group(int D, int K, int P, int Nm, int nR, int has_hset, int64_t B);
hipError_t launch_score_small(ScoreSmallArgs a, int D, hipStream_t st);
hipError_t small_read_trace(long long* host_dst, size_t n);

bool l2_tail_supported(int D);
hipError_t launch_l2_tail(const TailArgs& a, int D, hipStream_t st);
bool l2_tail_flash_applies(const TailArgs& a, int D);
hipError_t launch_l2_tail_flash(const TailArgs& a, hipStream_t st);
bool fused_l2_supported(int D, int K);
hipError_t launch_gather_attn_l2(const FusedL2Args& a, int D, int table_bf16, hipStream_t st);
bool fused_split_supported(int D, int K);
bool fused_split_applies(const FusedL2Args& a, int D);
hipError_t launch_gather_probe_l2(const void* table, const int32_t* ids1, const int32_t* ids2, int64_t n_parents, int K,
                                  int D, int table_bf16, float* sums, hipStream_t st);
hipError_t launch_group_pairs(const int64_t* u64, const int32_t* u32, int64_t B, int n_user, int32_t* count, int32_t* offs,
                              int32_t* rank, int32_t* seg_user, int32_t* seg_ptr, int32_t* nseg, int32_t* pair_index, hipStream_t st);
hipError_t launch_count_ids(const int32_t* ids, int64_t n, int nbins, float* out, hipStream_t st);
bool fused_d32_supported(int D, int K);
bool fused_d32_applies(const FusedL2Args& a, int D);
bool topk_rows_supported(int k);
hipError_t launch_topk_rows(const float* scores, int64_t rows, int64_t n, int64_t ld, const int32_t* cand_ids, int64_t col_offset,
                            const int64_t* excl_ptr, const int32_t* excl_ids, const int32_t* carry_ids, const float* carry_vals, int k,
                            int32_t* out_ids, float* out_vals, hipStream_t st);
hipError_t launch_rank_positives(const float* scores, int64_t rows, int64_t n, int64_t ld, const int32_t* cand_ids, int64_t col_offset,
                                 const int64_t* excl_ptr, const int32_t* excl_ids, const int64_t* pos_ptr, const int32_t* pos_ids,
                                 int32_t* out_counts, float* out_vals, int32_t* out_eligible, hipStream_t st);
int64_t ctr_counts_ws_bytes(int64_t n_seg, int64_t seg_len);
hipError_t launch_ctr_counts(const float* scores, const int32_t* labels, int64_t n_seg, int64_t seg_len, int64_t ld, void* ws,
                             int64_t* out, hipStream_t st);
bool sample_negatives_supported(int n_item);
hipError_t launch_sample_negatives(const int64_t* excl_ptr, const int32_t* excl_ids, const int32_t* counts, const int64_t* out_ptr,
                                   int n_user, int n_item, uint64_t seed, uint64_t round, int32_t* out, int64_t* status, hipStream_t st);
int64_t kg_explore_ws_bytes(int n_entity, int64_t M);
hipError_t launch_kg_field(const int64_t* eptr, const int32_t* edst, const int32_t* erel, int n_entity, int64_t M,
                           const int32_t* seeds, int64_t n_seed, int hops, void* ws, uint32_t* field_bits, int64_t* out_counts,
                           hipStream_t st);
hipError_t launch_kg_explore(const int64_t* eptr, const int32_t* edst, const int32_t* erel, int n_entity, int64_t M,
                             const int32_t* adj_entity, const int32_t* adj_relation, int K, const int32_t* seeds, int64_t n_seed,
                             int hops, void* ws, uint32_t* explored_bits, int64_t* out_counts, hipStream_t st);
size_t order_ws_elems(int64_t B);
hipError_t launch_order_by_key(const int64_t* k64, const int32_t* k32, int64_t B, int32_t* ws, int32_t* order, hipStream_t st);
bool fused_wpp_supported(int D, int K);
bool fused_wpp_applies(const FusedL2Args& a, int D);
hipError_t launch_gather_attn_l2_wpp(const FusedL2Args& a, hipStream_t st);
bool fused_agg_supported(int D, int K);
bool fused_fold_supported(int D, int K);
size_t fused_fold_lds_bytes(int D, int nR, int K);
bool fused_agg_applies(const FusedL2Args& a, int D);
hipError_t launch_entity_aggregates(const EntityAggArgs& a, hipStream_t st);
hipError_t launch_fold_prepare(const float* W0, const float* b0, const float* W1, const float* b1, const float* W2, const float* b2, const float* A0,
                               const float* a0, const float* Wmix, const float* bmix, const float* A1, float c, int D, float* blk, hipStream_t st);
hipError_t launch_l2_tail_fold(const TailFoldArgs& a, hipStream_t st);
hipError_t launch_score_l2_folded(const float* agg, const float* M0, const int32_t* adj_e, const int32_t* adj_r, const int32_t* items, int pid_stride,
                                  const float* t1, const float* q, const float* user_o, const float* Wq, const float* bq, const float* Wv,
                                  const float* bv, const float* Wqm, const float* A1, const float* a1, const float* Wm1, const float* Wm2,
                                  const float* bm, float* item_emb, float* scores, float* sig, int64_t B, int K, int D, int nR, int n_entity,
                                  hipStream_t st);
hipError_t launch_gather_attn_l2_agg(const FusedL2Args& a, hipStream_t st);
hipError_t launch_gather_attn_l2_d32(const FusedL2Args& a, int table_bf16, hipStream_t st, bool encoded = false);
bool fused_d16_supported(int D, int K);
bool fused_d16_applies(const FusedL2Args& a, int D);
hipError_t launch_gather_attn_l2_d16(const FusedL2Args& a, int table_bf16, hipStream_t st);
bool fused_l2_split_in_use();
hipError_t launch_gather_attn_l2_split(const FusedL2Args& a, int D, int table_bf16, hipStream_t st);
hipError_t split_read_trace(long long* host_dst, size_t n);
bool fused_packed_supported(int D, int K);
bool key_addr_static_er_ok(int P, int Nm, int nR, int n_entity, bool has_set);
hipError_t launch_transpose_blocks(const float* R, int nR, int D, float* RT, hipStream_t st);
constexpr int kEtMaxJobs = 24;
struct EntityTableJob {
    const float* W;
    float* out;
    int w_nk;
};
hipError_t launch_entity_tables(const float* E, int n_entity, const EntityTableJob* jobs, int njobs, hipStream_t st);
hipError_t launch_entity_dot(const float* E, const float* w, int n, int D, float* out, hipStream_t st);
hipError_t launch_prj_prepare(const float* W1, const float* W2, const float* b1, const float* b2, const float* A0, const float* a0,
                              float c, int D, float* blk, hipStream_t st);
bool fused_packed_applies(const FusedL2Args& a, int D);
hipError_t pack_read_prof(long long* host_dst, size_t n);
hipError_t launch_gather_attn_l2_packed(const FusedL2Args& a, int D, int table_bf16, hipStream_t st);
hipError_t launch_encode_adjacency(const int32_t* adj_e, const int32_t* adj_r, int n_entity, int K, int32_t* cnt,
                                   int32_t* enc_e, int32_t* enc_r, hipStream_t st);
hipError_t ka_read_trace(long long* host_dst, size_t n);

}
```

Baseline: 534.3 million.

## Software-pipeline folded L2 scoring kernel with prefetch and double-buffered neighbor lists

Restructures the folded hop-2 scoring kernel so the next batch's item id and query row are prefetched, and the first quad's adjacency loads, M0 and user rows are issued during the tail of the dense matmul chains. When LDS fits, a second per-wave neighbor-list buffer lets one list be built while the previous one is gathered. The launcher now picks between the pipelined single- and double-buffer variants by occupancy, and relation ids are clamped to the table size. It also adds an env-gated cycle-trace mode. The extra registers and LDS can lower occupancy.

```diff
diff --git a/mvin_amd/csrc/mvin_abi.hip b/mvin_amd/csrc/mvin_abi.hip
--- a/mvin_amd/csrc/mvin_abi.hip
+++ b/mvin_amd/csrc/mvin_abi.hip
@@ -80,6 +80,7 @@
     static const bool pk = getenv("MVIN_PACK_TRACE") != nullptr;
     if (getenv("MVIN_SMALL_TRACE")) return (int)mvin::small_read_trace(host_dst, n);
     if (getenv("MVIN_KAF_TRACE")) return (int)mvin::kaf_read_trace(host_dst, n);
+    if (getenv("MVIN_FOLD_TRACE")) return (int)mvin::fold_read_trace(host_dst, n);
     if (pk) return (int)mvin::pack_read_prof(host_dst, n);
     if (ka && getenv("MVIN_KA_TRACE")[0] == '2') return (int)mvin::kas_read_trace(host_dst, n);
     return (int)(ka ? mvin::ka_read_trace(host_dst, n) : mvin::split_read_trace(host_dst, n));
diff --git a/mvin_amd/csrc/mvin_fused_agg.h b/mvin_amd/csrc/mvin_fused_agg.h
--- a/mvin_amd/csrc/mvin_fused_agg.h
+++ b/mvin_amd/csrc/mvin_fused_agg.h
@@ -17,6 +17,7 @@
 constexpr unsigned kAggOob = 0xFFFFFFF0u;
 constexpr unsigned kAggPadRow = 0xFFFFFE00u;
 constexpr int agg_list_words(int K) { return 4 * 2 * (K + kAggPad); }
+constexpr size_t fused_agg_lds_words(int nR, int K) { return (size_t)((nR + 3) & ~3) + (size_t)kAggWaves * (16 * kAggUvLd + agg_list_words(K)); }
 size_t fused_agg_lds_bytes(int nR, int K);
 
 __device__ __forceinline__ int agg_xor16_imax(int v) {
@@ -47,13 +48,13 @@
 }
 
 template <int SPL, bool FAST, int LG = 4>
-__device__ __forceinline__ void agg_row_weights(const unsigned (&cr)[SPL], bool att, const float* sT, float invK, float (&wk)[SPL]) {
+__device__ __forceinline__ void agg_row_weights(const unsigned (&cr)[SPL], bool att, const float* sT, unsigned rmax, float invK, float (&wk)[SPL]) {
     float lg[SPL];
     float mx = -INFINITY;
 #pragma unroll
     for (int i = 0; i < SPL; ++i) {
         const float mu = (float)((cr[i] >> 16) & 0xFFu);
-        const float l = att ? sT[cr[i] & 0xFFFFu] : (FAST ? 1.f : 0.f);
+        const float l = att ? sT[min(cr[i] & 0xFFFFu, rmax)] : (FAST ? 1.f : 0.f);
         if constexpr (FAST) {
             wk[i] = mu * l;
         } else {
diff --git a/mvin_amd/csrc/mvin_fused_agg.hip b/mvin_amd/csrc/mvin_fused_agg.hip
--- a/mvin_amd/csrc/mvin_fused_agg.hip
+++ b/mvin_amd/csrc/mvin_fused_agg.hip
@@ -42,7 +42,7 @@
             const float4 sg = agg_row4(selfG, so);
             const float4 ss = agg_row4(selfS, so);
             float wk[SPL];
-            agg_row_weights<SPL, FAST>(cr, att, sT, invK, wk);
+            agg_row_weights<SPL, FAST>(cr, att, sT, (unsigned)(a.nR - 1), invK, wk);
             int cc = (int)(cr[0] >> 24);
             cc = valid ? (cc < 1 ? 1 : (cc > K ? K : cc)) : 0;
             __builtin_amdgcn_fence(__ATOMIC_RELEASE, "wavefront");
@@ -199,7 +199,7 @@
                 const float4 u1 = *reinterpret_cast<const float4*>(sUV + j * kAggUvLd + 4 * c);
                 const float4 vv = *reinterpret_cast<const float4*>(sUV + j * kAggUvLd + D + 4 * c);
                 float wk[SPL];
-                agg_row_weights<SPL, FAST>(cr, att1, sT, invK, wk);
+                agg_row_weights<SPL, FAST>(cr, att1, sT, (unsigned)(a.nR - 1), invK, wk);
                 int cc = (int)(cr[0] >> 24);
                 cc = pvalid ? (cc < 1 ? 1 : (cc > K ? K : cc)) : 0;
                 __builtin_amdgcn_fence(__ATOMIC_RELEASE, "wavefront");
@@ -265,20 +265,26 @@
     else run(std::false_type{});
 }
 
-template <int K>
+constexpr int kFoldTraceBatches = 16, kFoldTraceSlots = 20;
+__device__ long long g_fold_trace[kFoldTraceBatches * kFoldTraceSlots];
+
+template <int K, int MODE, bool TRACE = false>
 __global__ __launch_bounds__(kAggWaves * 64, 3) void score_l2_folded_kernel(FoldArgs a) {
     constexpr int D = 64, SPL = K / 16;
+    constexpr bool PIPE = MODE > 0, db = MODE == 2;
+    constexpr int lb = db ? agg_list_words(K) : 0;
     static_assert(K == 16 || K == 32 || K == 64, "K");
     extern __shared__ __attribute__((aligned(16))) float smem[];
     const int nRp = (a.nR + 3) & ~3;
     float* sT = smem;
-    const int tid = threadIdx.x, lane = tid & 63, wave = tid >> 6;
+    const int tid = threadIdx.x, lane = tid & 63, wave = __builtin_amdgcn_readfirstlane(tid >> 6);
     const int g = lane >> 4, c = lane & 15;
-    float* sUV = sT + nRp + wave * (16 * kAggUvLd + agg_list_words(K));
+    float* sUV = sT + nRp + wave * (16 * kAggUvLd + agg_list_words(K) + lb);
     unsigned* sLo = reinterpret_cast<unsigned*>(sUV + 16 * kAggUvLd) + g * (K + kAggPad);
     float* sLw = reinterpret_cast<float*>(reinterpret_cast<unsigned*>(sUV + 16 * kAggUvLd) + 4 * (K + kAggPad)) + g * (K + kAggPad);
     const bool att1 = a.t1 != nullptr;
     const float invK = 1.f / (float)K;
+    const unsigned rmax = (unsigned)(a.nR - 1);
     const bool fast = agg_logit_table(a.t1, a.nR, sT, tid, lane);
     __syncthreads();
 
@@ -289,31 +295,57 @@
     const __amdgpu_buffer_rsrc_t adjR = __builtin_amdgcn_make_buffer_rsrc(const_cast<int32_t*>(a.adj_r), 0, (int)a.adj_bytes, 0x00020000);
     const unsigned c16 = (unsigned)c * 16u;
     if (c < kAggPad) {
-        sLo[K + c] = kAggPadRow;
-        sLw[K + c] = 0.f;
+        sLo[K + c] = kAggPadRow, sLo[lb + K + c] = kAggPadRow;
+        sLw[K + c] = 0.f, sLw[lb + K + c] = 0.f;
     }
 
     const int64_t nbatch = (a.B + 15) >> 4;
     const int64_t nwaves = (int64_t)gridDim.x * kAggWaves;
+    int traced = 0;
+    auto stamp = [&](int slot, bool drain) {
+        if constexpr (TRACE) {
+            if (drain) asm volatile("s_waitcnt vmcnt(0)" ::: "memory");
+            if (blockIdx.x == 0 && tid == 0 && traced < kFoldTraceBatches) g_fold_trace[traced * kFoldTraceSlots + slot] = __builtin_readcyclecounter();
+        }
+    };
     auto run = [&](auto fast_tag) {
         constexpr bool FAST = decltype(fast_tag)::value;
+        const int lane = (int)__builtin_amdgcn_mbcnt_hi(~0u, __builtin_amdgcn_mbcnt_lo(~0u, 0u)), g = lane >> 4, c = lane & 15;
+        unsigned* sLo = reinterpret_cast<unsigned*>(sUV + 16 * kAggUvLd) + g * (K + kAggPad);
+        float* sLw = reinterpret_cast<float*>(reinterpret_cast<unsigned*>(sUV + 16 * kAggUvLd) + 4 * (K + kAggPad)) + g * (K + kAggPad);
+        const unsigned c16 = (unsigned)c * 16u;
+        unsigned xn = 0;
+        f32x4 qn[4];
+        auto fetch_batch = [&](int64_t b) {
+            const int64_t prn = min((min(b, nbatch - 1) << 4) + c, a.B - 1);
+            xn = (unsigned)a.items[prn * a.pid_stride];
+            const char* qrow = reinterpret_cast<const char*>(a.q) + (size_t)((unsigned)prn * (unsigned)(D * 4) + (unsigned)g * 16u);
+#pragma unroll
+            for (int nt = 0; nt < 4; ++nt) qn[nt] = *reinterpret_cast<const f32x4*>(qrow + 64 * nt);
+        };
+        if constexpr (PIPE) fetch_batch((int64_t)blockIdx.x * kAggWaves + wave);
         for (int64_t batch = (int64_t)blockIdx.x * kAggWaves + wave; batch < nbatch; batch += nwaves) {
             const int64_t p_base = batch << 4;
+            stamp(0, false);
             const int64_t pr = min(p_base + c, a.B - 1);
             const bool cvalid = p_base + c < a.B;
-            unsigned x0u = (unsigned)a.items[pr * a.pid_stride];
+            unsigned x0u;
+            if constexpr (PIPE) x0u = xn;
+            else x0u = (unsigned)a.items[pr * a.pid_stride];
             x0u = x0u < a.max_id ? x0u : a.max_id;
             const int x0c = (int)x0u;
             unsigned woff = ((unsigned)(4 * g) * (unsigned)D + (unsigned)c * 4u) * 4u;
             unsigned boff = (unsigned)g * 16u;
             unsigned roff = (unsigned)pr * (unsigned)(D * 4) + (unsigned)g * 16u;
             asm volatile("" : "+v"(woff), "+v"(boff));
-            auto chain3 = [&](const float* W0p, const float* W1p, const float* W2p, const f32x4 (&b0)[4], const f32x4 (&b1)[4], const f32x4 (&b2)[4],
-                              f32x4 (&acc0)[4], f32x4 (&acc1)[4], f32x4 (&acc2)[4], auto&& between) {
-                asm volatile("" : "+s"(W0p), "+s"(W1p), "+s"(W2p));
-                const __amdgpu_buffer_rsrc_t wr[3] = {__builtin_amdgcn_make_buffer_rsrc(const_cast<float*>(W0p), 0, D * D * 4, 0x00020000),
-                                                      __builtin_amdgcn_make_buffer_rsrc(const_cast<float*>(W1p), 0, D * D * 4, 0x00020000),
-                                                      __builtin_amdgcn_make_buffer_rsrc(const_cast<float*>(W2p), 0, D * D * 4, 0x00020000)};
+            auto chain = [&](auto np_, auto&& wsel, auto&& bsel, auto&& asel, auto&& between, auto&& late) {
+                constexpr int NP = decltype(np_)::value, T = 4 * NP;
+                __amdgpu_buffer_rsrc_t wr[NP];
+                static_for<NP>([&](auto j_) {
+                    const float* Wp = wsel(j_);
+                    asm volatile("" : "+s"(Wp));
+                    wr[decltype(j_)::value] = __builtin_amdgcn_make_buffer_rsrc(const_cast<float*>(Wp), 0, D * D * 4, 0x00020000);
+                });
                 f32x4 ring[3][4];
                 auto load = [&](auto s_) {
                     constexpr int s = decltype(s_)::value, j = s / 4, nt = s % 4;
@@ -325,12 +357,13 @@
                 };
                 load(std::integral_constant<int, 0>{});
                 load(std::integral_constant<int, 1>{});
-                static_for<12>([&](auto s_) {
+                static_for<T>([&](auto s_) {
                     constexpr int s = decltype(s_)::value, j = s / 4, nt = s % 4;
-                    if constexpr (s + 2 < 12) load(std::integral_constant<int, s + 2>{});
+                    if constexpr (s + 2 < T) load(std::integral_constant<int, s + 2>{});
+                    if constexpr (s >= T - 3) late(std::integral_constant<int, s - (T - 3)>{});
                     __builtin_amdgcn_sched_barrier(0);
-                    const f32x4 (&b)[4] = j == 0 ? b0 : j == 1 ? b1 : b2;
-                    f32x4 (&acc)[4] = j == 0 ? acc0 : j == 1 ? acc1 : acc2;
+                    const f32x4 (&b)[4] = bsel(std::integral_constant<int, j>{});
+                    f32x4 (&acc)[4] = asel(std::integral_constant<int, j>{});
 #pragma unroll
                     for (int r = 0; r < 4; ++r) {
 #pragma unroll
@@ -346,30 +379,6 @@
                 for (int ntp = 0; ntp < 4; ++ntp)
                     acc[ntp] = bias ? *reinterpret_cast<const f32x4*>(bias + 64 * ntp + (size_t)boff) : f32x4{0.f, 0.f, 0.f, 0.f};
             };
-            f32x4 qm[4], qb[4];
-            {
-                const char* qbase = reinterpret_cast<const char*>(a.q);
-#pragma unroll
-                for (int nt = 0; nt < 4; ++nt) qb[nt] = *reinterpret_cast<const f32x4*>(qbase + 64 * nt + (size_t)roff);
-                f32x4 at[4], av[4];
-                bias4(a.bq, at);
-                bias4(a.bv, av);
-                bias4(a.bm, qm);
-                if (!(a.dbg & 4))
-                    chain3(a.Wq, a.Wv, a.Wqm, qb, qb, qb, at, av, qm, [&](auto j_) {
-                        constexpr int j = decltype(j_)::value;
-                        if constexpr (j < 2) {
-                            const f32x4 (&acc)[4] = j == 0 ? at : av;
-#pragma unroll
-                            for (int ntp = 0; ntp < 4; ++ntp) *reinterpret_cast<f32x4*>(sUV + c * kAggUvLd + j * D + 16 * ntp + 4 * g) = acc[ntp];
-                        }
-                    });
-            }
-            __builtin_amdgcn_fence(__ATOMIC_RELEASE, "wavefront");
-            __builtin_amdgcn_wave_barrier();
-            __builtin_amdgcn_fence(__ATOMIC_ACQUIRE, "wavefront");
-
-            const int nquad = (a.dbg & 8) ? 0 : (int)((min((int64_t)16, a.B - p_base) + 3) >> 2);
             struct Quad {
                 unsigned ce[SPL], cr[SPL];
                 float4 s0;
@@ -381,93 +390,236 @@
                 qd.s0 = agg_row4(aggS, x0 * (unsigned)(D * 4) + c16);
                 return qd;
             };
-            Quad nx = quad_load(0);
-            for (int it = 0; it < nquad; ++it) {
-                const int j = 4 * it + g;
-                const bool pvalid = p_base + j < a.B;
-                const Quad qd = nx;
-                if (it + 1 < nquad) nx = quad_load(it + 1);
-                const unsigned (&ce)[SPL] = qd.ce;
-                const unsigned (&cr)[SPL] = qd.cr;
-                float* rowT = sUV + j * kAggUvLd + 4 * c;
-                const float4 tt = *reinterpret_cast<const float4*>(rowT);
-                const float4 vv = *reinterpret_cast<const float4*>(rowT + D);
+            Quad q0, q1;
+            auto late1 = [&](auto s_) {
+                if constexpr (PIPE && decltype(s_)::value == 0) q0 = quad_load(0), q1 = quad_load(1);
+            };
+            f32x4 qm[4], qb[4];
+            {
+                const char* qbase = reinterpret_cast<const char*>(a.q);
+#pragma unroll
+                for (int nt = 0; nt < 4; ++nt) {
+                    if constexpr (PIPE) qb[nt] = qn[nt];
+                    else qb[nt] = *reinterpret_cast<const f32x4*>(qbase + 64 * nt + (size_t)roff);
+                }
+                stamp(1, true);
+                f32x4 at[4], av[4];
+                bias4(a.bq, at);
+                bias4(a.bv, av);
+                auto store_tv = [&](auto j_) {
+                    constexpr int j = decltype(j_)::value;
+                    if constexpr (j < 2) {
+                        const f32x4 (&acc)[4] = j == 0 ? at : av;
+#pragma unroll
+                        for (int ntp = 0; ntp < 4; ++ntp) *reinterpret_cast<f32x4*>(sUV + c * kAggUvLd + j * D + 16 * ntp + 4 * g) = acc[ntp];
+                    }
+                };
+                bias4(a.bm, qm);
+                if (a.dbg & 4) late1(std::integral_constant<int, 0>{});
+                else
+                    chain(std::integral_constant<int, 3>{}, [&](auto j_) { return decltype(j_)::value == 0 ? a.Wq : decltype(j_)::value == 1 ? a.Wv : a.Wqm; },
+                          [&](auto) -> const f32x4 (&)[4] { return qb; },
+                          [&](auto j_) -> f32x4 (&)[4] {
+                              if constexpr (decltype(j_)::value == 0) return at;
+                              else if constexpr (decltype(j_)::value == 1) return av;
+                              else return qm;
+                          }, store_tv, late1);
+            }
+            __builtin_amdgcn_fence(__ATOMIC_RELEASE, "wavefront");
+            __builtin_amdgcn_wave_barrier();
+            __builtin_amdgcn_fence(__ATOMIC_ACQUIRE, "wavefront");
+            stamp(2, false);
+
+            const int nquad = (a.dbg & 8) ? 0 : (int)((min((int64_t)16, a.B - p_base) + 3) >> 2);
+            auto issue = [&](const unsigned* lo, int k, float4 (&r)[4]) {
+                const uint4 o4 = *reinterpret_cast<const uint4*>(lo + k);
+                r[0] = agg_row4(aggG, o4.x + c16), r[1] = agg_row4(aggG, o4.y + c16);
+                r[2] = agg_row4(aggG, o4.z + c16), r[3] = agg_row4(aggG, o4.w + c16);
+            };
+            auto sum4 = [&](const float4 (&r)[4], const float4& w, const f32x2 v01, const f32x2 v23, f32x2& a01, f32x2& a23) {
+                const float ws_[4] = {w.x, w.y, w.z, w.w};
+#pragma unroll
+                for (int t = 0; t < 4; ++t) {
+                    const f32x2 o01 = f32x2{r[t].x, r[t].y} + v01, o23 = f32x2{r[t].z, r[t].w} + v23;
+                    const f32x2 w2 = {ws_[t], ws_[t]};
+                    a01 = __builtin_elementwise_fma(w2, f32x2{fmaxf(o01[0], 0.f), fmaxf(o01[1], 0.f)}, a01);
+                    a23 = __builtin_elementwise_fma(w2, f32x2{fmaxf(o23[0], 0.f), fmaxf(o23[1], 0.f)}, a23);
+                }
+            };
+            auto lists = [&](const Quad& qd, int it, int ob) -> int {
+                const bool pvalid = p_base + 4 * it + g < a.B;
                 float wk[SPL];
-                agg_row_weights<SPL, FAST>(cr, att1, sT, invK, wk);
-                int cc = (int)(cr[0] >> 24);
+                agg_row_weights<SPL, FAST>(qd.cr, att1, sT, rmax, invK, wk);
+                int cc = (int)(qd.cr[0] >> 24);
                 cc = pvalid ? (cc < 1 ? 1 : (cc > K ? K : cc)) : 0;
                 __builtin_amdgcn_fence(__ATOMIC_RELEASE, "wavefront");
                 __builtin_amdgcn_wave_barrier();
 #pragma unroll
                 for (int i = 0; i < SPL; ++i) {
-                    sLo[SPL * c + i] = ((cr[i] >> 16) & 0xFFu) ? (ce[i] & 0xFFFFFFu) * (unsigned)(D * 4) : kAggPadRow;
-                    sLw[SPL * c + i] = wk[i];
+                    sLo[ob + SPL * c + i] = ((qd.cr[i] >> 16) & 0xFFu) ? (qd.ce[i] & 0xFFFFFFu) * (unsigned)(D * 4) : kAggPadRow;
+                    sLw[ob + SPL * c + i] = wk[i];
                 }
                 __builtin_amdgcn_fence(__ATOMIC_RELEASE, "wavefront");
                 __builtin_amdgcn_wave_barrier();
                 __builtin_amdgcn_fence(__ATOMIC_ACQUIRE, "wavefront");
-                const int kmax = (a.dbg & 1) ? 0 : __builtin_amdgcn_readfirstlane(agg_xor32_imax(agg_xor16_imax(cc)));
-                const f32x2 v01 = {vv.x, vv.y}, v23 = {vv.z, vv.w};
-                f32x2 a01 = {0.f, 0.f}, a23 = {0.f, 0.f};
-                float4 ra[4], rb[4];
-                float4 wa, wb;
-                auto issue = [&](int k, float4 (&r)[4], float4& w) {
-                    const uint4 o4 = *reinterpret_cast<const uint4*>(sLo + k);
-                    w = *reinterpret_cast<const float4*>(sLw + k);
-                    r[0] = agg_row4(aggG, o4.x + c16), r[1] = agg_row4(aggG, o4.y + c16);
-                    r[2] = agg_row4(aggG, o4.z + c16), r[3] = agg_row4(aggG, o4.w + c16);
-                };
-                auto sum4 = [&](const float4 (&r)[4], const float4& w) {
-                    const float ws_[4] = {w.x, w.y, w.z, w.w};
-#pragma unroll
-                    for (int t = 0; t < 4; ++t) {
-                        const f32x2 o01 = f32x2{r[t].x, r[t].y} + v01, o23 = f32x2{r[t].z, r[t].w} + v23;
-                        const f32x2 w2 = {ws_[t], ws_[t]};
-                        a01 = __builtin_elementwise_fma(w2, f32x2{fmaxf(o01[0], 0.f), fmaxf(o01[1], 0.f)}, a01);
-                        a23 = __builtin_elementwise_fma(w2, f32x2{fmaxf(o23[0], 0.f), fmaxf(o23[1], 0.f)}, a23);
+                return (a.dbg & 1) ? 0 : __builtin_amdgcn_readfirstlane(agg_xor32_imax(agg_xor16_imax(cc)));
+            };
+            if constexpr (PIPE) {
+                int kmax = lists(q0, 0, 0);
+                for (int it = 0; it < nquad; ++it) {
+                    stamp(3 + 3 * it, false);
+                    const int cur = (it & 1) ? lb : 0;
+                    float* rowT = sUV + (4 * it + g) * kAggUvLd + 4 * c;
+                    const float4 vv = *reinterpret_cast<const float4*>(rowT + D);
+                    const f32x2 v01 = {vv.x, vv.y}, v23 = {vv.z, vv.w};
+                    f32x2 a01 = {0.f, 0.f}, a23 = {0.f, 0.f};
+                    const int kr = (kmax + 7) & ~7;
+                    float4 r0[4], r1[4], r2[4];
+                    auto wts = [&](int k) { return *reinterpret_cast<const float4*>(sLw + cur + k); };
+                    const float4 s0 = q0.s0;
+                    if (it > 0 && it + 1 < nquad) q1 = quad_load(it + 1);
+                    issue(sLo + cur, 0, r0);
+                    issue(sLo + cur, 4, r1);
+                    if (kr > 8) issue(sLo + cur, 8, r2);
+                    stamp(4 + 3 * it, true);
+                    __builtin_amdgcn_sched_barrier(0);
+                    int kmax_n = 0;
+                    if (db && it + 1 < nquad) kmax_n = lists(q1, it + 1, lb - cur);
+                    __builtin_amdgcn_sched_barrier(0);
+                    for (int k0 = 0; k0 < kr; k0 += 24) {
+                        sum4(r0, wts(k0), v01, v23, a01, a23);
+                        __builtin_amdgcn_sched_barrier(0);
+                        if (k0 + 12 < kr) issue(sLo + cur, k0 + 12, r0);
+                        __builtin_amdgcn_sched_barrier(0);
+                        sum4(r1, wts(k0 + 4), v01, v23, a01, a23);
+                        __builtin_amdgcn_sched_barrier(0);
+                        if (k0 + 8 < kr) {
+                            if (k0 + 16 < kr) issue(sLo + cur, k0 + 16, r1);
+                            __builtin_amdgcn_sched_barrier(0);
+                            sum4(r2, wts(k0 + 8), v01, v23, a01, a23);
+                            __builtin_amdgcn_sched_barrier(0);
+                            if (k0 + 16 < kr) issue(sLo + cur, k0 + 20, r2);
+                            __builtin_amdgcn_sched_barrier(0);
+                            sum4(r0, wts(k0 + 12), v01, v23, a01, a23);
+                            __builtin_amdgcn_sched_barrier(0);
+                            if (k0 + 16 < kr) {
+                                if (k0 + 24 < kr) issue(sLo + cur, k0 + 24, r0);
+                                __builtin_amdgcn_sched_barrier(0);
+                                sum4(r1, wts(k0 + 16), v01, v23, a01, a23);
+                                __builtin_amdgcn_sched_barrier(0);
+                                if (k0 + 24 < kr) issue(sLo + cur, k0 + 28, r1);
+                                __builtin_amdgcn_sched_barrier(0);
+                                sum4(r2, wts(k0 + 20), v01, v23, a01, a23);
+                                __builtin_amdgcn_sched_barrier(0);
+                                if (k0 + 32 < kr) issue(sLo + cur, k0 + 32, r2);
+                                __builtin_amdgcn_sched_barrier(0);
+                            }
+                        }
                     }
-                };
-                issue(0, ra, wa);
-                for (int k0 = 0; k0 < kmax; k0 += 8) {
-                    issue(k0 + 4, rb, wb);
-                    __builtin_amdgcn_sched_barrier(0);
-                    sum4(ra, wa);
-                    __builtin_amdgcn_sched_barrier(0);
-                    issue(k0 + 8, ra, wa);
-                    __builtin_amdgcn_sched_barrier(0);
-                    sum4(rb, wb);
-                    __builtin_amdgcn_sched_barrier(0);
-                }
-                const float4 o0 = make_float4(fmaxf(qd.s0.x + tt.x, 0.f), fmaxf(qd.s0.y + tt.y, 0.f), fmaxf(qd.s0.z + tt.z, 0.f),
-                                              fmaxf(qd.s0.w + tt.w, 0.f));
-                *reinterpret_cast<float4*>(rowT) = o0;
-                *reinterpret_cast<float4*>(rowT + D) = make_float4(a01[0] + o0.x, a01[1] + o0.y, a23[0] + o0.z, a23[1] + o0.w);
+                    const float4 tt = *reinterpret_cast<const float4*>(rowT);
+                    const float4 o0 = make_float4(fmaxf(s0.x + tt.x, 0.f), fmaxf(s0.y + tt.y, 0.f), fmaxf(s0.z + tt.z, 0.f), fmaxf(s0.w + tt.w, 0.f));
+                    *reinterpret_cast<float4*>(rowT) = o0;
+                    *reinterpret_cast<float4*>(rowT + D) = make_float4(a01[0] + o0.x, a01[1] + o0.y, a23[0] + o0.z, a23[1] + o0.w);
+                    if (!db && it + 1 < nquad) kmax_n = lists(q1, it + 1, 0);
+                    kmax = kmax_n;
+                    q0 = q1;
+                    stamp(5 + 3 * it, false);
+                }
+            } else {
+                Quad nx = quad_load(0);
+                for (int it = 0; it < nquad; ++it) {
+                    stamp(3 + 3 * it, false);
+                    const Quad qd = nx;
+                    if (it + 1 < nquad) nx = quad_load(it + 1);
+                    float* rowT = sUV + (4 * it + g) * kAggUvLd + 4 * c;
+                    const float4 tt = *reinterpret_cast<const float4*>(rowT);
+                    const float4 vv = *reinterpret_cast<const float4*>(rowT + D);
+                    const int kmax = lists(qd, it, 0);
+                    const f32x2 v01 = {vv.x, vv.y}, v23 = {vv.z, vv.w};
+                    f32x2 a01 = {0.f, 0.f}, a23 = {0.f, 0.f};
+                    float4 ra[4], rb[4];
+                    float4 wa, wb;
+                    auto wts = [&](int k) { return *reinterpret_cast<const float4*>(sLw + k); };
+                    issue(sLo, 0, ra), wa = wts(0);
+                    if constexpr (TRACE) {
+                        issue(sLo, 4, rb), wb = wts(4);
+                        stamp(4 + 3 * it, true);
+                    }
+                    for (int k0 = 0; k0 < kmax; k0 += 8) {
+                        if (!TRACE || k0 > 0) issue(sLo, k0 + 4, rb), wb = wts(k0 + 4);
+                        __builtin_amdgcn_sched_barrier(0);
+                        sum4(ra, wa, v01, v23, a01, a23);
+                        __builtin_amdgcn_sched_barrier(0);
+                        issue(sLo, k0 + 8, ra), wa = wts(k0 + 8);
+                        __builtin_amdgcn_sched_barrier(0);
+                        sum4(rb, wb, v01, v23, a01, a23);
+                        __builtin_amdgcn_sched_barrier(0);
+                    }
+                    const float4 o0 = make_float4(fmaxf(qd.s0.x + tt.x, 0.f), fmaxf(qd.s0.y + tt.y, 0.f), fmaxf(qd.s0.z + tt.z, 0.f),
+                                                  fmaxf(qd.s0.w + tt.w, 0.f));
+                    *reinterpret_cast<float4*>(rowT) = o0;
+                    *reinterpret_cast<float4*>(rowT + D) = make_float4(a01[0] + o0.x, a01[1] + o0.y, a23[0] + o0.z, a23[1] + o0.w);
+                    stamp(5 + 3 * it, false);
+                }
             }
             __builtin_amdgcn_fence(__ATOMIC_RELEASE, "wavefront");
             __builtin_amdgcn_wave_barrier();
             __builtin_amdgcn_fence(__ATOMIC_ACQUIRE, "wavefront");
             {
-                f32x4 zb[4], ob[4], o2[4];
+                f32x4 zb[4], ob[4], o2[4], m0r[4], uor[4];
+                auto m0_load = [&]() {
+#pragma unroll
+                    for (int ntp = 0; ntp < 4; ++ntp)
+                        m0r[ntp] = *reinterpret_cast<const f32x4*>(reinterpret_cast<const char*>(a.M0) + (size_t)x0u * (D * 4) + 64 * ntp + (size_t)boff);
+                };
+                auto uo_load = [&]() {
+#pragma unroll
+                    for (int ntp = 0; ntp < 4; ++ntp)
+                        uor[ntp] = *reinterpret_cast<const f32x4*>(reinterpret_cast<const char*>(a.user_o) + 64 * ntp + (size_t)roff);
+                };
+                auto late2 = [&](auto s_) {
+                    if constexpr (PIPE && decltype(s_)::value == 0) m0_load();
+                    if constexpr (PIPE && decltype(s_)::value == 1) fetch_batch(batch + nwaves);
+                    if constexpr (PIPE && decltype(s_)::value == 2) uo_load();
+                };
 #pragma unroll
                 for (int nt = 0; nt < 4; ++nt) zb[nt] = *reinterpret_cast<const f32x4*>(sUV + c * kAggUvLd + D + 16 * nt + 4 * g);
                 bias4(a.a1, o2);
-                if (!(a.dbg & 2))
-                    chain3(a.A1, a.Wm1, a.Wm2, zb, ob, o2, o2, qm, qm, [&](auto j_) {
-                        if constexpr (decltype(j_)::value == 0) {
-#pragma unroll
-                            for (int nt = 0; nt < 4; ++nt) {
-                                o2[nt] = f32x4{fmaxf(o2[nt][0], 0.f), fmaxf(o2[nt][1], 0.f), fmaxf(o2[nt][2], 0.f), fmaxf(o2[nt][3], 0.f)};
-                                ob[nt] = *reinterpret_cast<const f32x4*>(sUV + c * kAggUvLd + 16 * nt + 4 * g);
-                            }
-                        }
-                    });
-                const bool uo_is_q = a.user_o == a.q;
+                auto relu_o2 = [&]() {
+#pragma unroll
+                    for (int nt = 0; nt < 4; ++nt) o2[nt] = f32x4{fmaxf(o2[nt][0], 0.f), fmaxf(o2[nt][1], 0.f), fmaxf(o2[nt][2], 0.f), fmaxf(o2[nt][3], 0.f)};
+                };
+                auto read_ob = [&]() {
+#pragma unroll
+                    for (int nt = 0; nt < 4; ++nt) ob[nt] = *reinterpret_cast<const f32x4*>(sUV + c * kAggUvLd + 16 * nt + 4 * g);
+                };
+                if (a.dbg & 2) late2(std::integral_constant<int, 0>{}), late2(std::integral_constant<int, 1>{}), late2(std::integral_constant<int, 2>{});
+                else
+                    chain(std::integral_constant<int, 3>{}, [&](auto j_) { constexpr int j = decltype(j_)::value; return j == 0 ? a.A1 : j == 1 ? a.Wm1 : a.Wm2; },
+                          [&](auto j_) -> const f32x4 (&)[4] {
+                              constexpr int j = decltype(j_)::value;
+                              if constexpr (j == 0) return zb;
+                              else if constexpr (j == 1) return ob;
+                              else return o2;
+                          },
+                          [&](auto j_) -> f32x4 (&)[4] { if constexpr (decltype(j_)::value == 0) return o2; else return qm; },
+                          [&](auto j_) {
+                              if constexpr (decltype(j_)::value == 0) relu_o2(), read_ob();
+                          }, late2);
+                stamp(15, false);
+                if constexpr (!PIPE) m0_load();
+                stamp(16, true);
+                if constexpr (!PIPE) {
+                    if (a.user_o != a.q) uo_load();
+                    else
+#pragma unroll
+                        for (int ntp = 0; ntp < 4; ++ntp) uor[ntp] = qb[ntp];
+                }
                 float part = 0.f;
 #pragma unroll
                 for (int ntp = 0; ntp < 4; ++ntp) {
-                    const f32x4 m0 = *reinterpret_cast<const f32x4*>(reinterpret_cast<const char*>(a.M0) + (size_t)x0u * (D * 4) + 64 * ntp + (size_t)boff);
-                    const f32x4 uo = uo_is_q ? qb[ntp] : *reinterpret_cast<const f32x4*>(reinterpret_cast<const char*>(a.user_o) + 64 * ntp + (size_t)roff);
-                    const f32x4 it4 = qm[ntp] + m0;
+                    const f32x4 uo = uor[ntp];
+                    const f32x4 it4 = qm[ntp] + m0r[ntp];
                     if (a.item_emb && cvalid) *reinterpret_cast<f32x4*>(reinterpret_cast<char*>(a.item_emb) + 64 * ntp + (size_t)roff) = it4;
                     part += it4[0] * uo[0] + it4[1] * uo[1] + it4[2] * uo[2] + it4[3] * uo[3];
                 }
@@ -476,31 +628,76 @@
                     a.scores[pr] = part;
                     if (a.sig) a.sig[pr] = 1.f / (1.f + expf(-part));
                 }
+                stamp(17, false);
             }
             __builtin_amdgcn_fence(__ATOMIC_RELEASE, "wavefront");
             __builtin_amdgcn_wave_barrier();
             __builtin_amdgcn_fence(__ATOMIC_ACQUIRE, "wavefront");
+            if constexpr (TRACE) ++traced;
         }
     };
     if (fast) run(std::true_type{});
     else run(std::false_type{});
 }
 
+hipError_t fold_read_trace(long long* host_dst, size_t n) {
+    const size_t have = sizeof(g_fold_trace) / sizeof(long long);
+    return hipMemcpyFromSymbol(host_dst, HIP_SYMBOL(g_fold_trace), (n < have ? n : have) * sizeof(long long));
+}
+
 template <int K>
 static hipError_t launch_fold_k(const FoldArgs& a, hipStream_t st) {
-    const size_t lds = fused_agg_lds_bytes(a.nR, K);
-    static thread_local int per_cu = 0;
-    if (per_cu == 0) {
-        int v = 0;
-        if (hipOccupancyMaxActiveBlocksPerMultiprocessor(&v, reinterpret_cast<const void*>(score_l2_folded_kernel<K>), kAggWaves * 64, lds) != hipSuccess || v < 1)
-            v = 4;
-        per_cu = v > 8 ? 8 : v;
-        if (const char* e = getenv("MVIN_FOLD_WGS")) per_cu = atoi(e) > 0 ? atoi(e) : per_cu;
+    static const bool pipe = !(getenv("MVIN_FOLD_PIPE") && atoi(getenv("MVIN_FOLD_PIPE")) == 0);
+    static const bool trace = getenv("MVIN_FOLD_TRACE") != nullptr;
+    static const int grid_cap = getenv("MVIN_FOLD_GRID") ? atoi(getenv("MVIN_FOLD_GRID")) : 0;
+    static const int wgs = getenv("MVIN_FOLD_WGS") ? atoi(getenv("MVIN_FOLD_WGS")) : 0;
+    using Kern = void (*)(FoldArgs);
+    constexpr size_t kLdsNoOptIn = 48 * 1024;
+    constexpr bool kTwoLists = fused_agg_lds_words(0, K) * sizeof(float) + (size_t)kAggWaves * agg_list_words(K) * sizeof(float) <= kLdsNoOptIn;
+    auto kernel_of = [&](int mode) -> Kern {
+        if (trace) {
+            if constexpr (kTwoLists) {
+                if (mode == 2) return score_l2_folded_kernel<K, 2, true>;
+            }
+            return mode ? (Kern)score_l2_folded_kernel<K, 1, true> : (Kern)score_l2_folded_kernel<K, 0, true>;
+        }
+        if constexpr (kTwoLists) {
+            if (mode == 2) return score_l2_folded_kernel<K, 2, false>;
+        }
+        return mode ? (Kern)score_l2_folded_kernel<K, 1, false> : (Kern)score_l2_folded_kernel<K, 0, false>;
+    };
+    struct Plan {
+        int dev, nR, per_cu;
+        size_t lds;
+        Kern kern;
+    };
+    static thread_local Plan plan{-1, -1, 0, 0, nullptr};
+    int dev = 0;
+    if (hipGetDevice(&dev) != hipSuccess) return hipGetLastError();
+    if (plan.dev != dev || plan.nR != a.nR) {
+        auto occupancy = [&](Kern k, size_t lds) {
+            int v = 0;
+            if (hipOccupancyMaxActiveBlocksPerMultiprocessor(&v, reinterpret_cast<const void*>(k), kAggWaves * 64, lds) != hipSuccess || v < 1) v = 0;
+            return v > 8 ? 8 : v;
+        };
+        const size_t lds1 = fused_agg_lds_bytes(a.nR, K), lds2 = lds1 + (size_t)kAggWaves * agg_list_words(K) * sizeof(float);
+        const int mode1 = pipe ? 1 : 0;
+        const int occ1 = occupancy(kernel_of(mode1), lds1);
+        const int occ2 = pipe && kTwoLists && lds2 <= kLdsNoOptIn ? occupancy(kernel_of(2), lds2) : 0;
+        const bool two = occ2 > 0 && occ2 >= occ1;
+        plan.kern = kernel_of(two ? 2 : mode1);
+        plan.lds = two ? lds2 : lds1;
+        plan.per_cu = two ? occ2 : occ1 > 0 ? occ1 : 4;
+        if (wgs > 0) plan.per_cu = wgs;
+        plan.dev = dev, plan.nR = a.nR;
+        if (getenv("MVIN_FOLD_REPORT"))
+            fprintf(stderr, "score_l2_folded_kernel<%d>: mode %d, LDS %zu bytes per workgroup, %d workgroups per CU\n", K, two ? 2 : mode1, plan.lds, plan.per_cu);
     }
     const int64_t nbatch = (a.B + 15) >> 4;
     const int64_t want = (nbatch + kAggWaves - 1) / kAggWaves;
-    const int64_t cap = 256 * (int64_t)per_cu;
-    score_l2_folded_kernel<K><<<(int)(want < cap ? want : cap), kAggWaves * 64, lds, st>>>(a);
+    int64_t cap = 256 * (int64_t)plan.per_cu;
+    if (grid_cap > 0 && grid_cap < cap) cap = grid_cap;
+    plan.kern<<<(int)(want < cap ? want : cap), kAggWaves * 64, plan.lds, st>>>(a);
     return hipGetLastError();
 }
 
@@ -530,9 +727,7 @@
 size_t fused_fold_d32_lds_bytes(int nR, int K);
 size_t fused_fold_lds_bytes(int D, int nR, int K) { return D == 32 ? fused_fold_d32_lds_bytes(nR, K) : fused_agg_lds_bytes(nR, K); }
 
-size_t fused_agg_lds_bytes(int nR, int K) {
-    return ((size_t)((nR + 3) & ~3) + (size_t)kAggWaves * (16 * kAggUvLd + agg_list_words(K))) * sizeof(float);
-}
+size_t fused_agg_lds_bytes(int nR, int K) { return fused_agg_lds_words(nR, K) * sizeof(float); }
 
 bool fused_agg_applies(const FusedL2Args& a, int D) {
     return a.prj && fused_agg_supported(D, a.K) && !a.probs_parent && !a.probs_child && a.adj_r && a.adj_bytes > 0 &&
diff --git a/mvin_amd/csrc/mvin_fused_agg32.hip b/mvin_amd/csrc/mvin_fused_agg32.hip
--- a/mvin_amd/csrc/mvin_fused_agg32.hip
+++ b/mvin_amd/csrc/mvin_fused_agg32.hip
@@ -50,7 +50,7 @@
             const float4 sg = agg_row4(selfG, so);
             const float4 ss = agg_row4(selfS, so);
             float wk[SPL];
-            agg_row_weights<SPL, FAST, 3>(cr, att, sT, invK, wk);
+            agg_row_weights<SPL, FAST, 3>(cr, att, sT, (unsigned)(a.nR - 1), invK, wk);
             int cc = (int)(cr[0] >> 24);
             cc = valid ? (cc < 1 ? 1 : (cc > K ? K : cc)) : 0;
             __builtin_amdgcn_fence(__ATOMIC_RELEASE, "wavefront");
@@ -226,7 +226,7 @@
                 const float4 tt = *reinterpret_cast<const float4*>(rowT);
                 const float4 vv = *reinterpret_cast<const float4*>(rowT + D);
                 float wk[SPL];
-                agg_row_weights<SPL, FAST, 3>(cr, att1, sT, invK, wk);
+                agg_row_weights<SPL, FAST, 3>(cr, att1, sT, (unsigned)(a.nR - 1), invK, wk);
                 int cc = (int)(cr[0] >> 24);
                 cc = pvalid ? (cc < 1 ? 1 : (cc > K ? K : cc)) : 0;
                 __builtin_amdgcn_fence(__ATOMIC_RELEASE, "wavefront");
diff --git a/mvin_amd/csrc/mvin_kernels.h b/mvin_amd/csrc/mvin_kernels.h
--- a/mvin_amd/csrc/mvin_kernels.h
+++ b/mvin_amd/csrc/mvin_kernels.h
@@ -353,6 +353,7 @@
 hipError_t launch_key_addr_flash(const KaFlashArgs& a, int nseg_bound, bool has_set, int32_t* sched_ws, hipStream_t st);
 hipError_t kas_read_trace(long long* host_dst, size_t n);
 hipError_t kaf_read_trace(long long* host_dst, size_t n);
+hipError_t fold_read_trace(long long* host_dst, size_t n);
 hipError_t launch_key_addr(const KeyAddrArgs& a, int table_bf16, hipStream_t st);
 bool key_addr_stream_supported(const KeyAddrArgs& a, int table_bf16);
 hipError_t launch_key_addr_stream(const KeyAddrArgs& a, int table_bf16, hipStream_t st);
```

Measured after the change: 545.5 million (median of 6 runs). 2.1% higher.
